# Yeicor/sdf-viewer

Hardware: AMD Instinct MI355X
Metric: Mvoxels/s grid fill + Mrays/s sphere-trace @1080p, demo SDF (higher is better)
Workload: dtype f32

## Files before the change

sdf-viewer_amd/csrc/api_march.hip:

```cpp
#include <cmath>
#include <cstddef>
#include <cstring>

#include "api_internal.h"
#include "march_common.h"
#include "raymarch_kernels.h"

using namespace sdfv;

namespace {

struct BatchStreams {
    static constexpr int kSide = 3;
    hipStream_t side[kSide] = {};
    hipEvent_t fork = nullptr, join[kSide] = {};
    int device = -1;
    void release() {
        for (int i = 0; i < kSide; ++i) {
            if (side[i]) (void)hipStreamDestroy(side[i]);
            if (join[i]) (void)hipEventDestroy(join[i]);
        }
        if (fork) (void)hipEventDestroy(fork);
        *this = BatchStreams{};
    }
    hipError_t ensure(int device_now) {
        if (device == device_now && fork) return hipSuccess;
        release();
        hipError_t e = hipEventCreateWithFlags(&fork, hipEventDisableTiming);
        for (int i = 0; i < kSide && e == hipSuccess; ++i) {
            e = hipStreamCreateWithFlags(&side[i], hipStreamNonBlocking);
            if (e == hipSuccess) e = hipEventCreateWithFlags(&join[i], hipEventDisableTiming);
        }
        if (e != hipSuccess) release();
        else device = device_now;
        return e;
    }
};
thread_local BatchStreams g_batch_streams;

struct CameraRing {
    static constexpr uint32_t kSlots = 16;
    sdfv_camera* base = nullptr;
    hipEvent_t read[kSlots] = {};
    bool recorded[kSlots] = {};
    uint32_t next = 0;
    int device = -1;
    void release() {
        for (uint32_t i = 0; i < kSlots; ++i)
            if (read[i]) (void)hipEventDestroy(read[i]);
        if (base) (void)hipFree(base);
        *this = CameraRing{};
    }
    hipError_t ensure(int device_now) {
        if (device == device_now && base) return hipSuccess;
        release();
        hipError_t e = hipMalloc(reinterpret_cast<void**>(&base), (size_t)kSlots * sdfv::kMaxCamerasPerLaunch * sizeof(sdfv_camera));
        for (uint32_t i = 0; i < kSlots && e == hipSuccess; ++i) e = hipEventCreateWithFlags(&read[i], hipEventDisableTiming);
        if (e != hipSuccess) {
            (void)hipGetLastError();
            release();
        } else {
            device = device_now;
        }
        return e;
    }
};
thread_local CameraRing g_camera_ring;

}

namespace sdfv {
void release_march_caches() {
    g_batch_streams.release();
    g_camera_ring.release();
}

int check_lights(const sdfv_render_params* rp) {
    if (rp->n_lights > SDFV_MAX_LIGHTS)
        return set_error(SDFV_ERR_INVALID_ARGUMENT, "n_lights %u exceeds SDFV_MAX_LIGHTS", rp->n_lights);
    for (uint32_t i = 0; i < rp->n_lights; ++i) {
        if (rp->lights[i].kind == SDFV_LIGHT_DIRECTIONAL)
            return set_error(SDFV_ERR_INVALID_ARGUMENT,
                        "lights[%u] is directional: three-d 0.18.2 shader source not available (scene/mod.rs:107-112 keeps "
                        "its directional lights commented out; their BRDF is not restated from memory)", i);
        if (rp->lights[i].kind != SDFV_LIGHT_AMBIENT)
            return set_error(SDFV_ERR_INVALID_ARGUMENT, "lights[%u] has unknown kind %u", i, rp->lights[i].kind);
    }
    return SDFV_OK;
}
}

namespace {

void derive_raymarch_args(const sdfv_render_params* rp, sdfv::RaymarchArgs& a) {
    memset(&a, 0, sizeof(a));
    a.rp = *rp;
    const uint32_t off = g_options.raymarch_disable;
    a.pow2_extent = (off & SDFV_RM_NO_POW2_EXTENT) ? 0u : 1u;
    a.fast_index = (off & SDFV_RM_NO_FAST_INDEX) ? 0u : 1u;
    a.pow2_size = 1;
    a.symmetric_box = 1;
    a.fast_normal = 1;
    float radius2 = 0.0f;
    const float h_world = sdfv::march::tap_distance((float)rp->tex_size[0], (float)rp->tex_size[1], (float)rp->tex_size[2],
                                                    rp->lod_dist_between_samples);
    for (int i = 0; i < 3; ++i) {
        a.bsize[i] = rp->bounds_max[i] - rp->bounds_min[i];
        a.inv_bsize[i] = 1.0f / a.bsize[i];
        const float n = (float)rp->tex_size[i];
        if (!(a.bsize[i] > 0.0f) || !(1e-4f * n / a.bsize[i] <= 0.25f)) a.fast_index = 0;
        if (!(a.bsize[i] > 0.0f) || !((1e-4f + h_world) * n / a.bsize[i] <= 0.45f)) a.fast_normal = 0;
        int e = 0;
        if (!(a.bsize[i] > 0.0f) || frexpf(a.bsize[i], &e) != 0.5f || e < -100 || e > 100) a.pow2_extent = 0;
        if (rp->tex_size[i] >= (1u << 24)) a.pow2_size = 0;
        if (rp->bounds_min[i] != -rp->bounds_max[i]) a.symmetric_box = 0;
        a.cull_center[i] = 0.5f * (rp->bounds_min[i] + rp->bounds_max[i]);
        radius2 += 0.25f * a.bsize[i] * a.bsize[i];
    }
    a.cull_radius2 = radius2 * 1.0201f + 1e-12f;
    if (!(a.cull_radius2 > 0.0f) || !std::isfinite(a.cull_radius2)) a.cull_radius2 = INFINITY;
    a.asm_loop = (off & SDFV_RM_NO_ASM_LOOP) ? 0u : 1u;
    a.no_interior_fetch = (off & SDFV_RM_NO_INTERIOR_FETCH) ? 1u : 0u;
    a.cube_box = (a.symmetric_box && rp->bounds_max[0] == rp->bounds_max[1] && rp->bounds_max[1] == rp->bounds_max[2]) ? 1u : 0u;
    if (off & SDFV_RM_NO_SYMMETRIC) a.symmetric_box = 0;
    if (off & SDFV_RM_NO_POW2_SIZE) a.pow2_size = 0;
}

void set_march_frame(sdfv::RaymarchArgs& a, const float* tex0, const float* tex1, uint32_t width, uint32_t height, uint32_t y0, uint32_t y1) {
    a.tex0 = reinterpret_cast<const float4*>(tex0);
    a.tex1 = reinterpret_cast<const float4*>(tex1);
    a.width = width;
    a.height = height;
    a.y0 = y0;
    a.y1 = y1;
}

int raymarch_rows(const sdfv_march_desc& d, uint32_t y0, uint32_t y1, uint32_t band_step, uint32_t band_height, void* stream) {
    const sdfv_render_params* rp = d.rp;
    const uint32_t n_cameras = d.n_cameras, width = d.width, height = d.height;
    const sdfv_camera* cameras = d.cameras;
    if (!rp || !d.tex0 || !d.tex1) return set_error(SDFV_ERR_INVALID_ARGUMENT, "NULL argument");
    if (!d.rgba && !d.rgba8) return set_error(SDFV_ERR_INVALID_ARGUMENT, "no colour output: rgba and rgba8 are both NULL");
    if (int rc = check_lights(rp)) return rc;
    if (int rc = check_texel_alignment(d.tex0, d.tex1, d.rgba)) return rc;
    if (int rc = check_word_aligned("dist, depth, aux and rgba8", d.dist, d.depth, d.aux, d.rgba8)) return rc;
    if (((uintptr_t)d.pairs | (uintptr_t)d.ilv) & 7) return set_error(SDFV_ERR_INVALID_ARGUMENT, "pairs and ilv must be 8-byte aligned");
    if (n_cameras && !cameras) return set_error(SDFV_ERR_INVALID_ARGUMENT, "cameras is NULL");
    if (y0 > y1 || y1 > height) return set_error(SDFV_ERR_INVALID_ARGUMENT, "rows [%u,%u) outside height %u", y0, y1, height);
    if (rp->tex_size[0] == 0 || rp->tex_size[1] == 0 || rp->tex_size[2] == 0)
        return set_error(SDFV_ERR_INVALID_ARGUMENT, "empty texture");
    if (!(rp->lod_dist_between_samples >= 1.0f)) return set_error(SDFV_ERR_INVALID_ARGUMENT, "lod_dist_between_samples < 1");
    const uint32_t lod_filter = g_options.raymarch_lod_filter;
    if (lod_filter == 1 && rp->lod_dist_between_samples != 1.0f) {
        int e = 0;
        const float lod = rp->lod_dist_between_samples;
        if (!(lod >= 2.0f && lod <= 32768.0f) || frexpf(lod, &e) != 0.5f)
            return set_error(SDFV_ERR_INVALID_ARGUMENT,
                             "SDFV_OPT_RAYMARCH_LOD_FILTER 1: lod_dist_between_samples %g is not a power of two in [2, 32768]", (double)lod);
    }
    if ((uint64_t)rp->tex_size[0] * rp->tex_size[1] * rp->tex_size[2] >= (1ull << 32))
        return set_error(SDFV_ERR_INVALID_ARGUMENT, "texture too large for 32-bit texel indexing");
    if (int rc = need_device()) return rc;
    sdfv::RaymarchArgs a;
    derive_raymarch_args(rp, a);
    a.dist = d.dist;
    a.pairs = d.pairs;
    a.ilv = d.ilv;
    set_march_frame(a, d.tex0, d.tex1, width, height, y0, y1);
    a.band_skip = band_height * (band_step - 1u);
    a.band_shift = band_height == 8u ? 3u : 4u;
    a.rows_out = band_step > 1 ? sdfv_band_rows_ex(height, y0 / band_height, band_step, band_height) : y1 - y0;
    a.compute_normal = g_options.raymarch_keep_normal ? 1u : 0u;
    const uint32_t w = g_options.raymarch_waves_per_simd;
    a.waves_per_simd = w;
    a.box_first = g_options.raymarch_box_first;
    const DeviceFacts& dev = device_facts();
    if (!dev.gfx950) a.asm_loop = 0;
    a.wave_slots_per_simd_unit = dev.cus * 4u;
    a.last_level_cache_bytes = dev.last_level_cache_bytes;
    const bool xcd_order_ok = dev.xcds == 8;
    a.group_shift = g_options.raymarch_tile_group == 0 ? (n_cameras == 1 && xcd_order_ok ? sdfv::kGroupAuto : 0u)
                                                       : (g_options.raymarch_tile_group == 1 ? 0u : g_options.raymarch_tile_group - 1u);
    a.rotate_columns = g_options.raymarch_tile_group == 0 && xcd_order_ok ? 1u : 0u;
#ifdef SDFV_TUNING
    a.wave_timing = reinterpret_cast<unsigned long long*>(g_options.wave_timing);
    a.priority_map = reinterpret_cast<const unsigned char*>(g_options.priority_map);
    a.tile_order = n_cameras == 1 ? reinterpret_cast<const uint32_t*>(g_options.tile_order) : nullptr;
#endif
    const uint64_t pixels_per_cam = (uint64_t)a.rows_out * width;
    hipStream_t main = (hipStream_t)stream;
    const sdfv_camera* device_cameras = nullptr;
    bool ring = false;
    hipPointerAttribute_t attr;
    if (hipPointerGetAttributes(&attr, cameras) == hipSuccess && (attr.type == hipMemoryTypeDevice || attr.type == hipMemoryTypeManaged)) {
        device_cameras = cameras;
    } else {
        (void)hipGetLastError();
        if (n_cameras > sdfv::kInlineCameras) {
            hipStreamCaptureStatus capturing = hipStreamCaptureStatusNone;
            if (hipStreamIsCapturing(main, &capturing) != hipSuccess) (void)hipGetLastError();
            ring = capturing == hipStreamCaptureStatusNone && g_options.raymarch_camera_staging &&
                   g_camera_ring.ensure(current_device()) == hipSuccess;
        }
    }
    const uint32_t per_launch = device_cameras || ring ? sdfv::kMaxCamerasPerLaunch : sdfv::kInlineCameras;
    const uint64_t groups_per_launch = (uint64_t)((width + 15) / 16) * ((a.rows_out + 15) / 16) * per_launch;
    const bool overlap = n_cameras > per_launch && groups_per_launch <= 40000 && g_options.raymarch_batch_streams;
    uint32_t used = 0;
    int rc = SDFV_OK;
    auto hip_ok = [&](hipError_t e, const char* what) {
        if (e != hipSuccess && rc == SDFV_OK) rc = hip_fail(e, what);
        return e == hipSuccess;
    };
    if (overlap) hip_ok(g_batch_streams.ensure(current_device()), "batch streams") && hip_ok(hipEventRecord(g_batch_streams.fork, main), "hipEventRecord");
    uint32_t launch = 0;
    for (uint32_t c0 = 0; c0 < n_cameras && rc == SDFV_OK; c0 += per_launch, ++launch) {
        const uint32_t nc = n_cameras - c0 < per_launch ? n_cameras - c0 : per_launch;
        a.n_cameras = nc;
        if (device_cameras) a.camera_list = device_cameras + c0;
        else if (!ring) memcpy(a.cameras, cameras + c0, nc * sizeof(sdfv_camera));
        point_outputs_at(a, pixels_per_cam, c0, d.rgba, d.rgba8, d.aux, d.depth);
        hipStream_t on = main;
        const uint32_t lane = launch % (BatchStreams::kSide + 1);
        if (overlap && lane != 0) {
            on = g_batch_streams.side[lane - 1];
            if (lane > used) {
                if (!hip_ok(hipStreamWaitEvent(on, g_batch_streams.fork, 0), "hipStreamWaitEvent")) break;
                used = lane;
            }
        }
        if (ring) {
            CameraRing& r = g_camera_ring;
            const uint32_t slot = r.next++ % CameraRing::kSlots;
            sdfv_camera* at = r.base + (size_t)slot * sdfv::kMaxCamerasPerLaunch;
            if (r.recorded[slot] && !hip_ok(hipStreamWaitEvent(on, r.read[slot], 0), "hipStreamWaitEvent")) break;
            if (!hip_ok(sdfv::launch_store_cameras(cameras + c0, nc, at, on), "store_cameras")) break;
            a.camera_list = at;
            hip_ok(sdfv::launch_raymarch(a, on, lod_filter), "launch_raymarch") && hip_ok(hipEventRecord(r.read[slot], on), "hipEventRecord");
            r.recorded[slot] = true;
            continue;
        }
        hip_ok(sdfv::launch_raymarch(a, on, lod_filter), "launch_raymarch");
    }
    for (uint32_t i = 0; i < used; ++i)
        hip_ok(hipEventRecord(g_batch_streams.join[i], g_batch_streams.side[i]), "hipEventRecord") &&
            hip_ok(hipStreamWaitEvent(main, g_batch_streams.join[i], 0), "hipStreamWaitEvent");
    return rc;
}

int slab_round_args(const sdfv_render_params* rp, const sdfv_grid* slab, uint32_t ghost_lo, uint32_t ghost_hi,
                           const float* tex0, const float* tex1, const sdfv_camera* camera, uint32_t width, uint32_t height,
                           float* rgba, sdfv_march_aux* aux, sdfv::RaymarchArgs& a, sdfv::SlabMarchArgs& s) {
    if (!rp || !slab || !tex0 || !tex1 || !camera || !rgba) return set_error(SDFV_ERR_INVALID_ARGUMENT, "NULL argument");
    if (int rc = check_grid(slab)) return rc;
    if (int rc = check_lights(rp)) return rc;
    if (int rc = check_texel_alignment(tex0, tex1, rgba)) return rc;
    for (int i = 0; i < 3; ++i)
        if (rp->tex_size[i] != slab->dims[i])
            return set_error(SDFV_ERR_INVALID_ARGUMENT, "render parameters describe a %ux%ux%u grid, the slab a %ux%ux%u one",
                        rp->tex_size[0], rp->tex_size[1], rp->tex_size[2], slab->dims[0], slab->dims[1], slab->dims[2]);
    if (slab->z_begin >= slab->z_end) return set_error(SDFV_ERR_INVALID_ARGUMENT, "empty slab");
    if (ghost_lo > slab->z_begin || slab->z_end + ghost_hi > slab->dims[2])
        return set_error(SDFV_ERR_INVALID_ARGUMENT, "ghost slices reach outside the grid");
    if (ghost_lo > 1 || ghost_hi > 2) return set_error(SDFV_ERR_INVALID_ARGUMENT, "at most 1 lower and 2 upper ghost slices");
    if (slab->z_end < slab->dims[2] && ghost_hi == 0)
        return set_error(SDFV_ERR_INVALID_ARGUMENT, "an interior slab needs its upper ghost slice (run the halo exchange)");
    if (rp->lod_dist_between_samples != 1.0f)
        return set_error(SDFV_ERR_INVALID_ARGUMENT, "the sharded march renders loaded grids only (lod_dist_between_samples == 1)");
    if ((uint64_t)width * height >= (1ull << 32)) return set_error(SDFV_ERR_INVALID_ARGUMENT, "image too large");
    const uint64_t resident = (uint64_t)slab->dims[0] * slab->dims[1] * (ghost_lo + (slab->z_end - slab->z_begin) + ghost_hi);
    if (resident >= (1ull << 32)) return set_error(SDFV_ERR_INVALID_ARGUMENT, "slab too large for 32-bit texel indexing");
    if (int rc = need_device()) return rc;
    derive_raymarch_args(rp, a);
    if (!a.fast_index)
        return set_error(SDFV_ERR_INVALID_ARGUMENT, "box too small for the sharded march: 1e-4 * N / size must be <= 0.25");
    set_march_frame(a, tex0, tex1, width, height, 0, height);
    a.rows_out = height;
    a.band_shift = 4;
    a.n_cameras = 1;
    a.cameras[0] = *camera;
    a.rgba = reinterpret_cast<float4*>(rgba);
    a.aux = aux;
    s = sdfv::SlabMarchArgs{};
    s.z_lo = slab->z_begin - ghost_lo;
    s.z_count = ghost_lo + (slab->z_end - slab->z_begin) + ghost_hi;
    s.own_begin = slab->z_begin;
    s.own_end = slab->z_end;
    return SDFV_OK;
}

}

#pragma GCC visibility push(default)
extern "C" {

void sdfv_render_params_default(sdfv_render_params* rp, const sdfv_grid* grid) {
    if (!rp) return;
    memset(rp, 0, sizeof(*rp));
    for (int i = 0; i < 3; ++i) {
        if (grid) {
            rp->bounds_min[i] = grid->bb_min[i];
            rp->bounds_max[i] = grid->bb_max[i];
            rp->tex_size[i] = grid->dims[i];
        }
        rp->ambient[i] = 1.0f;
    }
    rp->lod_dist_between_samples = 1.0f;
    rp->tint[0] = rp->tint[1] = rp->tint[2] = rp->tint[3] = 1.0f;
    rp->gamma = 0.0f;
    rp->tone_mapping = 2;
    rp->color_mapping = 1;
}

int sdfv_march_volume_advice(const sdfv_grid* grid, uint32_t* kind) {
    if (int rc = check_grid(grid)) return rc;
    if (!kind) return set_error(SDFV_ERR_INVALID_ARGUMENT, "kind is NULL");
    if (int rc = need_device()) return rc;
    sdfv_render_params rp;
    sdfv_render_params_default(&rp, grid);
    sdfv::RaymarchArgs a;
    derive_raymarch_args(&rp, a);
    if (!device_facts().gfx950) a.asm_loop = 0;
    a.last_level_cache_bytes = device_facts().last_level_cache_bytes;
    const int mode = sdfv::march_volume_choice(a, true, true, true);
    *kind = mode == sdfv::kMarchIlv ? SDFV_MARCH_VOLUME_INTERLEAVED : mode == sdfv::kMarchPairs ? SDFV_MARCH_VOLUME_PAIRS : SDFV_MARCH_VOLUME_NONE;
    return SDFV_OK;
}

int sdfv_raymarch_ex(const sdfv_march_desc* desc, void* stream) {
    sdfv_march_desc d;
    if (int rc = read_sized_desc(desc, offsetof(sdfv_march_desc, depth), "sdfv_march_desc", d)) return rc;
    if (d.reserved != 0) return set_error(SDFV_ERR_INVALID_ARGUMENT, "sdfv_march_desc: reserved fields must be 0");
    if (d.band_step == 0 && d.band_height != 0)
        return set_error(SDFV_ERR_INVALID_ARGUMENT, "band_height %u with band_step 0: a band set needs band_step >= 1 (0 = rows [y0, y1))", d.band_height);
    if (d.band_step == 0)
        return raymarch_rows(d, d.y0, d.y1, 1, 16, stream);
    const uint32_t B = d.band_height ? d.band_height : 16u;
    if (B != 8u && B != 16u) return set_error(SDFV_ERR_INVALID_ARGUMENT, "band_height %u: 8 or 16 (0 = 16)", d.band_height);
    if (sdfv_band_rows_ex(d.height, d.band_first, d.band_step, B) == 0) return SDFV_OK;
    return raymarch_rows(d, d.band_first * B, d.height, d.band_step, B, stream);
}

uint32_t sdfv_band_rows_ex(uint32_t height, uint32_t band_first, uint32_t band_step, uint32_t band_height) {
    const uint32_t B = band_height ? band_height : 16u;
    if (B != 8u && B != 16u) return 0;
    const uint32_t bands = (height + B - 1) / B;
    if (band_step == 0 || band_first >= bands) return 0;
    const uint32_t n = (bands - band_first + band_step - 1) / band_step, last = band_first + (n - 1) * band_step;
    return (n - 1) * B + (height - last * B < B ? height - last * B : B);
}
uint32_t sdfv_band_rows(uint32_t height, uint32_t band_first, uint32_t band_step) {
    return sdfv_band_rows_ex(height, band_first, band_step, 16u);
}

int sdfv_raymarch_slab(const sdfv_render_params* rp, const sdfv_grid* slab, uint32_t ghost_lo, uint32_t ghost_hi,
                       const float* tex0, const float* tex1, const sdfv_camera* camera, uint32_t width, uint32_t height,
                       const sdfv_ray_state* in_states, uint32_t n_in, float* rgba, sdfv_march_aux* aux,
                       sdfv_ray_state* out_down, sdfv_ray_state* out_up, uint32_t capacity, uint32_t* counters,
                       void* stream) {
    if (!out_down || !out_up || !counters) return set_error(SDFV_ERR_INVALID_ARGUMENT, "NULL argument");
    if (in_states == nullptr && n_in != 0) return set_error(SDFV_ERR_INVALID_ARGUMENT, "n_in without in_states");
    sdfv::RaymarchArgs a;
    sdfv::SlabMarchArgs s;
    if (int rc = slab_round_args(rp, slab, ghost_lo, ghost_hi, tex0, tex1, camera, width, height, rgba, aux, a, s)) return rc;
    s.in = in_states;
    s.n_in = n_in;
    s.out_down = out_down;
    s.out_up = out_up;
    s.count_down = counters;
    s.count_up = counters + 1;
    s.capacity = capacity;
    if (in_states && n_in == 0) return SDFV_OK;
    SDFV_HIP_RETURN(sdfv::launch_raymarch_slab(a, s, (hipStream_t)stream));
}

size_t sdfv_ray_buffer_bytes(uint32_t capacity) { return SDFV_RAY_BUFFER_HEADER_BYTES + (size_t)capacity * sizeof(sdfv_ray_state); }

int sdfv_raymarch_slab_round(const sdfv_render_params* rp, const sdfv_grid* slab, uint32_t ghost_lo, uint32_t ghost_hi,
                             const float* tex0, const float* tex1, const sdfv_camera* camera, uint32_t width, uint32_t height,
                             const void* in_lo, const void* in_hi, int first_round, float* rgba, sdfv_march_aux* aux,
                             void* out_down, void* out_up, uint32_t capacity, uint32_t* overflow, void* stream) {
    return sdfv_internal_raymarch_slab_round(rp, slab, ghost_lo, ghost_hi, tex0, tex1, camera, width, height, in_lo, in_hi,
                                             first_round, rgba, aux, out_down, out_up, capacity, overflow, nullptr, stream);
}

__attribute__((visibility("hidden"))) int sdfv_internal_raymarch_slab_round(
    const sdfv_render_params* rp, const sdfv_grid* slab, uint32_t ghost_lo, uint32_t ghost_hi, const float* tex0, const float* tex1,
    const sdfv_camera* camera, uint32_t width, uint32_t height, const void* in_lo, const void* in_hi, int first_round, float* rgba,
    sdfv_march_aux* aux, void* out_down, void* out_up, uint32_t capacity, uint32_t* overflow, uint32_t* leftover, void* stream) {
    if (!out_down || !out_up) return set_error(SDFV_ERR_INVALID_ARGUMENT, "NULL ray buffer");
    if (int rc = check_word_aligned("ray buffers", in_lo, in_hi, out_down, out_up, overflow)) return rc;
    if (first_round && (in_lo || in_hi)) return set_error(SDFV_ERR_INVALID_ARGUMENT, "the first round takes no incoming rays");
    sdfv::RaymarchArgs a;
    sdfv::SlabMarchArgs s;
    if (int rc = slab_round_args(rp, slab, ghost_lo, ghost_hi, tex0, tex1, camera, width, height, rgba, aux, a, s)) return rc;
    auto count_of = [](const void* b) { return reinterpret_cast<const uint32_t*>(b); };
    auto rays_of = [](const void* b) {
        return reinterpret_cast<const sdfv_ray_state*>(static_cast<const char*>(b) + SDFV_RAY_BUFFER_HEADER_BYTES);
    };
    SDFV_HIP(hipMemsetAsync(out_down, 0, SDFV_RAY_BUFFER_HEADER_BYTES, (hipStream_t)stream));
    SDFV_HIP(hipMemsetAsync(out_up, 0, SDFV_RAY_BUFFER_HEADER_BYTES, (hipStream_t)stream));
    if (!first_round) {
        if (!in_lo && !in_hi) return SDFV_OK;
        s.in_count[0] = in_lo ? count_of(in_lo) : nullptr;
        s.in_rays[0] = in_lo ? rays_of(in_lo) : nullptr;
        s.in_count[1] = in_hi ? count_of(in_hi) : nullptr;
        s.in_rays[1] = in_hi ? rays_of(in_hi) : nullptr;
        const uint64_t most = (uint64_t)capacity * ((in_lo ? 1u : 0u) + (in_hi ? 1u : 0u));
        const uint64_t pixels = (uint64_t)width * height;
        s.max_in = (uint32_t)(most < pixels ? most : pixels);
        if (s.max_in == 0) return SDFV_OK;
    }
    s.out_down = const_cast<sdfv_ray_state*>(rays_of(out_down));
    s.out_up = const_cast<sdfv_ray_state*>(rays_of(out_up));
    s.count_down = reinterpret_cast<uint32_t*>(out_down);
    s.count_up = reinterpret_cast<uint32_t*>(out_up);
    s.overflow = overflow;
    s.leftover = leftover;
    s.capacity = capacity;
    SDFV_HIP_RETURN(sdfv::launch_raymarch_slab(a, s, (hipStream_t)stream));
}

}
#pragma GCC visibility pop
```

sdf-viewer_amd/csrc/raymarch_kernels.h:

```cpp
#pragma once

#include <hip/hip_runtime.h>
#include <stdint.h>

#include "../../include/sdfgrid.h"

namespace sdfv {

struct RaymarchArgs {
    sdfv_render_params rp;
    float bsize[3];
    float inv_bsize[3];
    uint32_t pow2_extent;
    uint32_t fast_index;
    const float* dist;
    const float* pairs;
    const float* ilv;
    uint32_t pow2_size;
    uint32_t symmetric_box;
    uint32_t fast_normal;
    float cull_center[3];
    float cull_radius2;
    const float4* tex0;
    const float4* tex1;
    uint32_t n_cameras;
    uint32_t width, height;
    uint32_t y0, y1;
    uint32_t compute_normal;
    uint32_t asm_loop;
    uint32_t group_shift;
    uint32_t tiles_x, tiles_y, groups_x;
    uint32_t box_first;
    uint32_t first_gx0, first_gy0, first_w, first_h, m_groups_x, m_first_w, m_rest_w;
    uint32_t no_interior_fetch;
    uint32_t rotate_columns;
    uint32_t lds_cap_bytes;
    uint32_t waves_per_simd;
    uint32_t wave_slots_per_simd_unit;
    uint64_t last_level_cache_bytes;
    uint32_t cube_box;
    uint32_t rows_out;
    uint32_t band_skip;
    uint32_t band_shift;
    float4* rgba;
    uint32_t* rgba8;
    sdfv_march_aux* aux;
    float* depth;
#ifdef SDFV_TUNING
    const uint32_t* tile_order;
    const unsigned char* priority_map;
    unsigned long long* wave_timing;
#endif
    const sdfv_camera* camera_list;
    sdfv_camera cameras[16];
};

constexpr int kMarchGeneral = 0, kMarchTex0 = 1, kMarchDist = 2, kMarchPairs = 3, kMarchIlv = 4, kMarchLattice = 5;

constexpr uint32_t kInlineCameras = 16;
constexpr uint32_t kMaxCamerasPerLaunch = 64;
constexpr uint32_t kGroupAuto = 255;

struct SlabMarchArgs {
    uint32_t z_lo, z_count;
    uint32_t own_begin, own_end;
    const sdfv_ray_state* in;
    uint32_t n_in;
    const uint32_t* in_count[2];
    const sdfv_ray_state* in_rays[2];
    uint32_t max_in;
    sdfv_ray_state* out_down;
    sdfv_ray_state* out_up;
    uint32_t* count_down;
    uint32_t* count_up;
    uint32_t* overflow;
    uint32_t* leftover;
    uint32_t capacity;
};
hipError_t launch_raymarch_slab(const RaymarchArgs& a, const SlabMarchArgs& s, hipStream_t stream);

hipError_t launch_raymarch(const RaymarchArgs& a, hipStream_t stream, uint32_t lod_filter);
bool march_volume_applicable(const RaymarchArgs& a, int kind);
int march_volume_choice(const RaymarchArgs& a, bool have_dist, bool have_pairs, bool have_ilv);
hipError_t launch_store_cameras(const sdfv_camera* host, uint32_t n, sdfv_camera* device, hipStream_t stream);

}
```

sdf-viewer_amd/csrc/raymarch_kernels.hip:

```cpp
#include "raymarch_kernels.h"

#include <hip/hip_runtime.h>
#include <string.h>

#include "march_common.h"

namespace sdfv {
namespace {

using namespace march;

__device__ __forceinline__ uint32_t mirror_index(int i, int n) {
    if (i >= 0 && i < n) return (uint32_t)i;
    int period = 2 * n;
    int m = i % period;
    if (m < 0) m += period;
    return (uint32_t)(m < n ? m : period - 1 - m);
}

struct Tex {
    const float4* data;
    int w, h, d;
    int z_lo;
};

struct Footprint {
    uint32_t o000, o100, o010, o110, o001, o101, o011, o111;
    float ax, ay, az;
};

constexpr int kMirror = 0, kClamp = 1, kClampSlab = 2;

template <int POLICY>
__device__ __forceinline__ Footprint footprint(const Tex& t, V3 p01, int& k0c) {
    float u = p01.x * (float)t.w - 0.5f, v = p01.y * (float)t.h - 0.5f, w = p01.z * (float)t.d - 0.5f;
    float fu = floorf(u), fv = floorf(v), fw = floorf(w);
    Footprint f;
    f.ax = u - fu; f.ay = v - fv; f.az = w - fw;
    int i0 = (int)fu, j0 = (int)fv, k0 = (int)fw;
    uint32_t i0m, i1m, j0m, j1m, k0m, k1m;
    const uint32_t sy = (uint32_t)t.w, sz = (uint32_t)t.w * (uint32_t)t.h;
    k0c = 0;
    if (POLICY == kMirror) {
        i0m = mirror_index(i0, t.w); i1m = mirror_index(i0 + 1, t.w);
        j0m = mirror_index(j0, t.h) * sy; j1m = mirror_index(j0 + 1, t.h) * sy;
        k0m = mirror_index(k0, t.d) * sz; k1m = mirror_index(k0 + 1, t.d) * sz;
    } else {
        const int z0 = POLICY == kClampSlab ? t.z_lo : 0;
        i0m = (uint32_t)max(i0, 0); i1m = (uint32_t)min(i0 + 1, t.w - 1);
        j0m = (uint32_t)max(j0, 0) * sy; j1m = (uint32_t)min(j0 + 1, t.h - 1) * sy;
        k0c = min(max(k0, 0), t.d - 1);
        k0m = (uint32_t)(max(k0, 0) - z0) * sz; k1m = (uint32_t)(min(k0 + 1, t.d - 1) - z0) * sz;
    }
    f.o000 = k0m + j0m + i0m; f.o100 = k0m + j0m + i1m;
    f.o010 = k0m + j1m + i0m; f.o110 = k0m + j1m + i1m;
    f.o001 = k1m + j0m + i0m; f.o101 = k1m + j0m + i1m;
    f.o011 = k1m + j1m + i0m; f.o111 = k1m + j1m + i1m;
    return f;
}

__device__ __forceinline__ float trilerp(float t000, float t100, float t010, float t110, float t001, float t101,
                                         float t011, float t111, float ax, float ay, float az) {
    float c00 = mixf(t000, t100, ax), c10 = mixf(t010, t110, ax);
    float c01 = mixf(t001, t101, ax), c11 = mixf(t011, t111, ax);
    return mixf(mixf(c00, c10, ay), mixf(c01, c11, ay), az);
}

template <int POLICY>
__device__ __forceinline__ Footprint footprint(const Tex& t, V3 p01) {
    int k0c;
    return footprint<POLICY>(t, p01, k0c);
}

__device__ __forceinline__ float gather_r(const float* base, uint32_t stride, const Footprint& f) {
    const float t000 = base[(uint64_t)f.o000 * stride], t100 = base[(uint64_t)f.o100 * stride];
    const float t010 = base[(uint64_t)f.o010 * stride], t110 = base[(uint64_t)f.o110 * stride];
    const float t001 = base[(uint64_t)f.o001 * stride], t101 = base[(uint64_t)f.o101 * stride];
    const float t011 = base[(uint64_t)f.o011 * stride], t111 = base[(uint64_t)f.o111 * stride];
    return trilerp(t000, t100, t010, t110, t001, t101, t011, t111, f.ax, f.ay, f.az);
}

__device__ __forceinline__ float4 gather_rgba(const float4* data, const Footprint& f) {
    const float4 t000 = data[f.o000], t100 = data[f.o100], t010 = data[f.o010], t110 = data[f.o110];
    const float4 t001 = data[f.o001], t101 = data[f.o101], t011 = data[f.o011], t111 = data[f.o111];
    float4 r;
    r.x = trilerp(t000.x, t100.x, t010.x, t110.x, t001.x, t101.x, t011.x, t111.x, f.ax, f.ay, f.az);
    r.y = trilerp(t000.y, t100.y, t010.y, t110.y, t001.y, t101.y, t011.y, t111.y, f.ax, f.ay, f.az);
    r.z = trilerp(t000.z, t100.z, t010.z, t110.z, t001.z, t101.z, t011.z, t111.z, f.ax, f.ay, f.az);
    r.w = trilerp(t000.w, t100.w, t010.w, t110.w, t001.w, t101.w, t011.w, t111.w, f.ax, f.ay, f.az);
    return r;
}

template <int XF>
__device__ __forceinline__ V3 to_p01(const RaymarchArgs& a, V3 p) {
    if (XF >= 1)
        return mk((p.x - a.rp.bounds_min[0]) * a.inv_bsize[0], (p.y - a.rp.bounds_min[1]) * a.inv_bsize[1],
                  (p.z - a.rp.bounds_min[2]) * a.inv_bsize[2]);
    return mk((p.x - a.rp.bounds_min[0]) / a.bsize[0], (p.y - a.rp.bounds_min[1]) / a.bsize[1],
              (p.z - a.rp.bounds_min[2]) / a.bsize[2]);
}

__device__ __forceinline__ uint32_t nearest_offset(const RaymarchArgs& a, const Tex& t, V3 p01) {
    float rx = (float)t.w / a.rp.lod_dist_between_samples;
    float ry = (float)t.h / a.rp.lod_dist_between_samples;
    float rz = (float)t.d / a.rp.lod_dist_between_samples;
    float qx = roundf(p01.x * rx) / rx, qy = roundf(p01.y * ry) / ry, qz = roundf(p01.z * rz) / rz;
    int i = (int)floorf(qx * (float)t.w), j = (int)floorf(qy * (float)t.h), k = (int)floorf(qz * (float)t.d);
    return (mirror_index(k, t.d) * (uint32_t)t.h + mirror_index(j, t.h)) * (uint32_t)t.w + mirror_index(i, t.w);
}

template <bool LINEAR, int XF, int POLICY>
__device__ __forceinline__ float sample_r(const RaymarchArgs& a, const float* __restrict__ base, uint32_t stride, const Tex& t, V3 p) {
    V3 q = to_p01<XF>(a, p);
    if (LINEAR) return gather_r(base, stride, footprint<POLICY>(t, q));
    return base[(uint64_t)nearest_offset(a, t, q) * stride];
}

template <bool LINEAR, int XF, int POLICY>
__device__ __forceinline__ float4 sample_rgba(const RaymarchArgs& a, const Tex& t, V3 p) {
    V3 q = to_p01<XF>(a, p);
    if (LINEAR) return gather_rgba(t.data, footprint<POLICY>(t, q));
    return t.data[nearest_offset(a, t, q)];
}

template <bool SYMM>
__device__ __forceinline__ float oob_dist(const RaymarchArgs& a, V3 p) {
    if (SYMM) {
        return fmaxf(fabsf(p.x) - a.rp.bounds_max[0],
                     fmaxf(fabsf(p.y) - a.rp.bounds_max[1], fabsf(p.z) - a.rp.bounds_max[2]));
    }
    return march::oob_dist(a.rp, p);
}

template <int MODE>
__device__ __forceinline__ const float* march_volume(const RaymarchArgs& a) {
    return MODE == kMarchTex0 ? reinterpret_cast<const float*>(a.tex0) : MODE == kMarchDist ? a.dist : MODE == kMarchPairs ? a.pairs : a.ilv;
}

template <int MODE, int XF, bool SYMM, bool T>
__device__ __forceinline__ void march_fast(const RaymarchArgs& a, const Tex& t, V3 ray_dir, bool covered, V3& ray_pos,
                                           float& dist_from_origin, int& status, int& steps, int& iterations) {
    static_assert(MODE == kMarchTex0 || MODE == kMarchDist, "the pair and interleaved volumes are read by the hand-written loop only");
    constexpr int STRIDE = MODE == kMarchTex0 ? 4 : 1;
    const float* __restrict__ vol = march_volume<MODE>(a);
    const float fw_ = (float)t.w, fh_ = (float)t.h, fd_ = (float)t.d;
    const float kx = a.inv_bsize[0] * fw_, ky = a.inv_bsize[1] * fh_, kz = a.inv_bsize[2] * fd_;
    const int wm1 = t.w - 1, hm1 = t.h - 1, dm1 = t.d - 1;
    const uint32_t sy = (uint32_t)t.w, sz = (uint32_t)t.w * (uint32_t)t.h;
    bool marching = covered;
    int last_i = -1;
    float cfu = -4.0f, cfv = -4.0f, cfw = -4.0f;
    float t000 = 0.0f, t100 = 0.0f, t010 = 0.0f, t110 = 0.0f, t001 = 0.0f, t101 = 0.0f, t011 = 0.0f, t111 = 0.0f;
    for (int i = 0; i < 255; ++i) {
        marching = marching && !(oob_dist<SYMM>(a, ray_pos) > 1e-4f);
        if (__ballot(marching) == 0ull) break;
        ++iterations;
        last_i = marching ? i : last_i;
        float u, v, w;
        if (XF == 2) {
            u = (ray_pos.x - a.rp.bounds_min[0]) * kx - 0.5f;
            v = (ray_pos.y - a.rp.bounds_min[1]) * ky - 0.5f;
            w = (ray_pos.z - a.rp.bounds_min[2]) * kz - 0.5f;
        } else {
            const V3 q = to_p01<XF>(a, ray_pos);
            u = q.x * fw_ - 0.5f; v = q.y * fh_ - 0.5f; w = q.z * fd_ - 0.5f;
        }
        const float fu = floorf(u), fv = floorf(v), fw = floorf(w);
        const float ax = u - fu, ay = v - fv, az = w - fw;
        if (marching && (fu != cfu || fv != cfv || fw != cfw)) {
            cfu = fu; cfv = fv; cfw = fw;
            const int i0 = (int)fu, j0 = (int)fv, k0 = (int)fw;
            const uint32_t i0c = (uint32_t)max(i0, 0), i1c = (uint32_t)min(i0 + 1, wm1);
            const uint32_t j0c = (uint32_t)max(j0, 0) * sy, j1c = (uint32_t)min(j0 + 1, hm1) * sy;
            const uint32_t k0c = (uint32_t)max(k0, 0) * sz, k1c = (uint32_t)min(k0 + 1, dm1) * sz;
            const uint32_t r00 = k0c + j0c, r10 = k0c + j1c, r01 = k1c + j0c, r11 = k1c + j1c;
            if (STRIDE == 1 && wm1 >= 1) {
                const uint32_t b = (uint32_t)min(max(i0, 0), wm1 - 1);
                const bool lo_is_x = i0c == b, hi_is_y = i1c == b + 1;
                typedef float f2 __attribute__((ext_vector_type(2), aligned(4)));
                const f2 q00 = *reinterpret_cast<const f2*>(vol + (uint64_t)(r00 + b));
                const f2 q10 = *reinterpret_cast<const f2*>(vol + (uint64_t)(r10 + b));
                const f2 q01 = *reinterpret_cast<const f2*>(vol + (uint64_t)(r01 + b));
                const f2 q11 = *reinterpret_cast<const f2*>(vol + (uint64_t)(r11 + b));
                t000 = lo_is_x ? q00.x : q00.y; t100 = hi_is_y ? q00.y : q00.x;
                t010 = lo_is_x ? q10.x : q10.y; t110 = hi_is_y ? q10.y : q10.x;
                t001 = lo_is_x ? q01.x : q01.y; t101 = hi_is_y ? q01.y : q01.x;
                t011 = lo_is_x ? q11.x : q11.y; t111 = hi_is_y ? q11.y : q11.x;
            } else {
                t000 = vol[(uint64_t)(r00 + i0c) * STRIDE]; t100 = vol[(uint64_t)(r00 + i1c) * STRIDE];
                t010 = vol[(uint64_t)(r10 + i0c) * STRIDE]; t110 = vol[(uint64_t)(r10 + i1c) * STRIDE];
                t001 = vol[(uint64_t)(r01 + i0c) * STRIDE]; t101 = vol[(uint64_t)(r01 + i1c) * STRIDE];
                t011 = vol[(uint64_t)(r11 + i0c) * STRIDE]; t111 = vol[(uint64_t)(r11 + i1c) * STRIDE];
            }
        }
        const float sample_dist = trilerp(t000, t100, t010, t110, t001, t101, t011, t111, ax, ay, az) - 1e-1f;
        marching = marching && !(sample_dist < 1e-5f);
        const V3 np = madd(ray_pos, ray_dir, sample_dist);
        ray_pos.x = marching ? np.x : ray_pos.x;
        ray_pos.y = marching ? np.y : ray_pos.y;
        ray_pos.z = marching ? np.z : ray_pos.z;
        if (T) {
            const float nt = dist_from_origin + sample_dist;
            dist_from_origin = marching ? nt : dist_from_origin;
        }
    }
    steps = last_i + 1;
    if (covered) status = marching ? -1 : (oob_dist<SYMM>(a, ray_pos) > 1e-4f ? -2 : 1);
}

struct Lattice {
    uint32_t shift;
    float inv_l;
    int mx1, my1, mz1;
};
__device__ __forceinline__ Lattice lattice_of(const RaymarchArgs& a, const Tex& t) {
    const uint32_t l = (uint32_t)a.rp.lod_dist_between_samples;
    Lattice g;
    g.shift = 31u - (uint32_t)__builtin_clz(l);
    g.inv_l = 1.0f / a.rp.lod_dist_between_samples;
    g.mx1 = (int)(((uint32_t)t.w + l - 1u) >> g.shift) - 1;
    g.my1 = (int)(((uint32_t)t.h + l - 1u) >> g.shift) - 1;
    g.mz1 = (int)(((uint32_t)t.d + l - 1u) >> g.shift) - 1;
    return g;
}
__device__ __forceinline__ void lattice_cell(const Tex& t, const Lattice& g, float fu, float fv, float fw, Footprint& f) {
    const int i0 = (int)fu, j0 = (int)fv, k0 = (int)fw;
    const uint32_t sy = (uint32_t)t.w, sz = (uint32_t)t.w * (uint32_t)t.h;
    const uint32_t i0m = (uint32_t)min(max(i0, 0), g.mx1) << g.shift, i1m = (uint32_t)min(max(i0 + 1, 0), g.mx1) << g.shift;
    const uint32_t j0m = ((uint32_t)min(max(j0, 0), g.my1) << g.shift) * sy, j1m = ((uint32_t)min(max(j0 + 1, 0), g.my1) << g.shift) * sy;
    const uint32_t k0m = ((uint32_t)min(max(k0, 0), g.mz1) << g.shift) * sz, k1m = ((uint32_t)min(max(k0 + 1, 0), g.mz1) << g.shift) * sz;
    f.o000 = k0m + j0m + i0m; f.o100 = k0m + j0m + i1m;
    f.o010 = k0m + j1m + i0m; f.o110 = k0m + j1m + i1m;
    f.o001 = k1m + j0m + i0m; f.o101 = k1m + j0m + i1m;
    f.o011 = k1m + j1m + i0m; f.o111 = k1m + j1m + i1m;
}
__device__ __forceinline__ Footprint lattice_footprint(const Tex& t, const Lattice& g, V3 p01) {
    const float u = p01.x * (float)t.w - 0.5f, v = p01.y * (float)t.h - 0.5f, w = p01.z * (float)t.d - 0.5f;
    const float su = u * g.inv_l, sv = v * g.inv_l, sw = w * g.inv_l;
    const float fu = floorf(su), fv = floorf(sv), fw = floorf(sw);
    Footprint f;
    f.ax = su - fu; f.ay = sv - fv; f.az = sw - fw;
    lattice_cell(t, g, fu, fv, fw, f);
    return f;
}

template <int XF, bool SYMM, bool T>
__device__ __forceinline__ void march_lattice(const RaymarchArgs& a, const Tex& t, const Lattice& g, V3 ray_dir, bool covered, V3& ray_pos,
                                              float& dist_from_origin, int& status, int& steps, int& iterations) {
    static_assert(XF == 0 || XF == 1, "no fused scale: s = (q * N - 0.5) / L keeps the LINEAR footprint's u");
    const float* __restrict__ vol = reinterpret_cast<const float*>(a.tex0);
    const float fw_ = (float)t.w, fh_ = (float)t.h, fd_ = (float)t.d;
    bool marching = covered;
    int last_i = -1;
    float cfu = __int_as_float(0x7fc00000), cfv = cfu, cfw = cfu;
    float t000 = 0.0f, t100 = 0.0f, t010 = 0.0f, t110 = 0.0f, t001 = 0.0f, t101 = 0.0f, t011 = 0.0f, t111 = 0.0f;
    for (int i = 0; i < 255; ++i) {
        marching = marching && !(oob_dist<SYMM>(a, ray_pos) > 1e-4f);
        if (__ballot(marching) == 0ull) break;
        ++iterations;
        last_i = marching ? i : last_i;
        const V3 q = to_p01<XF>(a, ray_pos);
        const float su = (q.x * fw_ - 0.5f) * g.inv_l, sv = (q.y * fh_ - 0.5f) * g.inv_l, sw = (q.z * fd_ - 0.5f) * g.inv_l;
        const float fu = floorf(su), fv = floorf(sv), fw = floorf(sw);
        const float ax = su - fu, ay = sv - fv, az = sw - fw;
        if (marching && (fu != cfu || fv != cfv || fw != cfw)) {
            cfu = fu; cfv = fv; cfw = fw;
            Footprint c;
            lattice_cell(t, g, fu, fv, fw, c);
            t000 = vol[(uint64_t)c.o000 * 4]; t100 = vol[(uint64_t)c.o100 * 4];
            t010 = vol[(uint64_t)c.o010 * 4]; t110 = vol[(uint64_t)c.o110 * 4];
            t001 = vol[(uint64_t)c.o001 * 4]; t101 = vol[(uint64_t)c.o101 * 4];
            t011 = vol[(uint64_t)c.o011 * 4]; t111 = vol[(uint64_t)c.o111 * 4];
        }
        const float sample_dist = trilerp(t000, t100, t010, t110, t001, t101, t011, t111, ax, ay, az) - 1e-1f;
        marching = marching && !(sample_dist < 1e-5f);
        const V3 np = madd(ray_pos, ray_dir, sample_dist);
        ray_pos.x = marching ? np.x : ray_pos.x;
        ray_pos.y = marching ? np.y : ray_pos.y;
        ray_pos.z = marching ? np.z : ray_pos.z;
        if (T) {
            const float nt = dist_from_origin + sample_dist;
            dist_from_origin = marching ? nt : dist_from_origin;
        }
    }
    steps = last_i + 1;
    if (covered) status = marching ? -1 : (oob_dist<SYMM>(a, ray_pos) > 1e-4f ? -2 : 1);
}

#ifdef SDFV_TUNING
#define SDFV_MARCH_ASM_TUNE(x) x
#else
#define SDFV_MARCH_ASM_TUNE(x) ""
#endif
#define SDFV_MARCH_ASM_HEAD(ROW_BYTES)                                                                                         \
    "s_mov_b64 s[76:77], exec\n"                                                                                    \
    "s_and_b64 exec, exec, %[cov]\n"                                                                                \
    "s_cbranch_execz .Ldone_%=\n"                                                                                   \
          \
    "s_mov_b32 s66, %[miny]\n s_mov_b32 s67, %[minz]\n"                                            \
    "s_mov_b32 s70, %[ky]\n s_mov_b32 s71, %[kz]\n"                                                    \
    "s_mov_b32 s72, 0xbf000000\n s_mov_b32 s73, 0xbf000000\n"                                      \
    "s_add_i32 s75, %[wm1], -1\n"                                                                         \
    "s_lshl_b32 s82, %[w], 2\n s_lshl_b32 s83, %[w], 4\n"         \
    "s_lshl_b32 s85, %[w], 3\n"                                      \
    "s_movk_i32 s74, 254\n"                                                                      \
     \
    "s_mov_b32 s64, " ROW_BYTES "\n"                                                                                 \
    "s_mul_i32 s86, %[h], " ROW_BYTES "\n"                                                                           \
    "s_add_u32 s68, %[base_lo], s86\n s_addc_u32 s69, %[base_hi], 0\n"                                      \
    "s_add_u32 s64, %[base_lo], s64\n s_addc_u32 s65, %[base_hi], 0\n"                                      \
    "s_add_u32 s86, s64, s86\n s_addc_u32 s87, s65, 0\n"                                                    \
    SDFV_MARCH_ASM_TUNE("s_mov_b32 s84, 0\n")                  \
    "v_mov_b32 v68, 0x7f800000\n v_mov_b32 v70, 0x7f800000\n v_mov_b32 v71, 0x7f800000\n"     \
    ".Lloop_%=:\n"
#define SDFV_MARCH_ASM_OOB4_A "v_sub_f32_e64 v32, |v40|, %[mx]\n"
#define SDFV_MARCH_ASM_OOB4_B "v_sub_f32_e64 v33, |v42|, %[my]\n"
#define SDFV_MARCH_ASM_OOB4_C "v_sub_f32_e64 v34, |v43|, %[mz]\n"
#define SDFV_MARCH_ASM_OOB4_D "v_max3_f32 v32, v32, v33, v34\n"
#define SDFV_MARCH_ASM_OOB2_A "v_max3_f32 v32, |v40|, |v42|, |v43|\n"
#define SDFV_MARCH_ASM_OOB2_D "v_subrev_f32_e32 v32, %[mx], v32\n"
#define SDFV_MARCH_ASM_TOP(T_STEP, OOB_A, OOB_B, OOB_C, OOB_D)                                                      \
    OOB_A                                                                                                           \
    "v_subrev_f32_e32 v48, %[minx], v40\n"                                                                          \
    OOB_B                                                                                                           \
    "v_pk_add_f32 v[50:51], v[42:43], s[66:67] neg_lo:[0,1] neg_hi:[0,1]\n"                                         \
    OOB_C                                                                                                           \
    "v_mul_f32_e32 v48, %[kx], v48\n"                                                                               \
    "v_pk_mul_f32 v[50:51], v[50:51], s[70:71]\n"                                                                   \
    OOB_D                                                                                                           \
    "v_add_f32_e32 v48, -0.5, v48\n"                                                                                \
    "v_pk_add_f32 v[50:51], v[50:51], s[72:73]\n"                                                                   \
    "v_cmpx_nlt_f32_e32 vcc, 0x38d1b717, v32\n"                                           \
    "s_cbranch_execz .Ldone_%=\n"                                                                                   \
    "v_sub_f32_e32 v52, v48, v68\n"                                                                              \
    "v_sub_f32_e32 v54, v50, v70\n"                                                                              \
    "v_sub_f32_e32 v56, v51, v71\n" T_STEP                                                                       \
    "v_max3_u32 v32, v52, v54, v56\n"                                                                            \
    "v_cmp_gt_u32_e32 vcc, 0x3f800000, v32\n"                                                                       \
    "s_andn1_saveexec_b64 s[78:79], vcc\n"                                      \
    "s_cbranch_execnz .Lfetch_%=\n"                                  \
    ".Lcached_%=:\n"
#define SDFV_MARCH_ASM_FETCH_PREP(INTERIOR)                                                                         \
    ".Lfetch_%=:\n"                                                                                                 \
    SDFV_MARCH_ASM_TUNE("s_add_u32 s84, s84, 1\n")                                                                  \
        \
    "v_floor_f32_e32 v68, v48\n v_floor_f32_e32 v70, v50\n v_floor_f32_e32 v71, v51\n"                         \
    "v_cvt_i32_f32_e32 v32, v68\n v_cvt_i32_f32_e32 v33, v70\n v_cvt_i32_f32_e32 v34, v71\n"                      \
    "v_sub_f32_e32 v52, v48, v68\n v_sub_f32_e32 v54, v50, v70\n v_sub_f32_e32 v56, v51, v71\n"             \
     \
    "v_max3_u32 v35, v32, v33, v34\n"                                                                               \
    "v_cmp_gt_u32_e32 vcc, %[thresh], v35\n"                                                                        \
    "s_xor_b64 vcc, vcc, exec\n"                                                                                    \
    "s_cbranch_scc1 .Lborder_%=\n"                                                                                  \
    "v_mad_u32_u24 v39, v34, %[h], v33\n"                     \
    "v_mad_u32_u24 v39, v39, %[w], v32\n" INTERIOR                                                               \
    "s_branch .Lcached_%=\n"                                                                                        \
    ".Lborder_%=:\n"                                                                                                \
    "v_max_i32_e32 v35, 0, v32\n v_max_i32_e32 v37, 0, v33\n v_max_i32_e32 v38, 0, v34\n"         \
    "v_add_u32_e32 v32, 1, v32\n v_add_u32_e32 v33, 1, v33\n v_add_u32_e32 v34, 1, v34\n"                            \
    "v_min_i32_e32 v32, %[wm1], v32\n v_min_i32_e32 v33, %[hm1], v33\n v_min_i32_e32 v34, %[dm1], v34\n"   \
    "v_mad_u32_u24 v28, v38, %[h], v37\n"                                                      \
    "v_mad_u32_u24 v29, v38, %[h], v33\n"                                                      \
    "v_mad_u32_u24 v30, v34, %[h], v37\n"                                                      \
    "v_mad_u32_u24 v31, v34, %[h], v33\n"
#define SDFV_MARCH_ASM_INTERIOR_DIST                                                                                \
    "v_lshlrev_b32_e32 v39, 2, v39\n"                                                                               \
    "global_load_dwordx2 v[24:25], v39, %[base]\n"                                        \
    "global_load_dwordx2 v[26:27], v39, s[64:65]\n"                                       \
    "global_load_dwordx2 v[28:29], v39, s[68:69]\n"                                       \
    "global_load_dwordx2 v[30:31], v39, s[86:87]\n"                                       \
    "s_waitcnt vmcnt(1)\n"                                                                                          \
    "v_pk_mov_b32 v[60:61], v[24:25], v[28:29] op_sel:[0,0]\n"                                    \
    "v_pk_mov_b32 v[62:63], v[24:25], v[28:29] op_sel:[1,1]\n"                                    \
    "s_waitcnt vmcnt(0)\n"                                                                                          \
    "v_pk_mov_b32 v[64:65], v[26:27], v[30:31] op_sel:[0,0]\n"                                    \
    "v_pk_mov_b32 v[66:67], v[26:27], v[30:31] op_sel:[1,1]\n"
#define SDFV_MARCH_ASM_INTERIOR_TEX0                                                                                \
    "v_lshlrev_b32_e32 v39, 4, v39\n"                                                                               \
    "global_load_dword v60, v39, %[base]\n global_load_dword v62, v39, %[base] offset:16\n"                       \
    "global_load_dword v64, v39, s[64:65]\n global_load_dword v66, v39, s[64:65] offset:16\n"                     \
    "global_load_dword v61, v39, s[68:69]\n global_load_dword v63, v39, s[68:69] offset:16\n"                     \
    "global_load_dword v65, v39, s[86:87]\n global_load_dword v67, v39, s[86:87] offset:16\n"                     \
    "s_waitcnt vmcnt(0)\n"
#define SDFV_MARCH_ASM_INTERIOR_PAIRS                                                                               \
    "v_lshlrev_b32_e32 v39, 3, v39\n"                                                                               \
    "global_load_dwordx4 v[24:27], v39, %[base]\n"                                  \
    "global_load_dwordx4 v[28:31], v39, s[68:69]\n"                                 \
    "s_waitcnt vmcnt(0)\n"                                                                                          \
    "v_pk_mov_b32 v[60:61], v[24:25], v[28:29] op_sel:[0,0]\n"                                    \
    "v_pk_mov_b32 v[64:65], v[24:25], v[28:29] op_sel:[1,1]\n"                                    \
    "v_pk_mov_b32 v[62:63], v[26:27], v[30:31] op_sel:[0,0]\n"                                    \
    "v_pk_mov_b32 v[66:67], v[26:27], v[30:31] op_sel:[1,1]\n"
#define SDFV_MARCH_ASM_FETCH_PAIRS                                                                                  \
    "v_lshlrev_b32_e32 v35, 3, v35\n v_lshlrev_b32_e32 v32, 3, v32\n"                  \
    "v_mad_u32_u24 v24, v28, s85, v35\n v_mad_u32_u24 v25, v28, s85, v32\n"                                          \
    "global_load_dword v60, v24, %[base]\n global_load_dword v62, v25, %[base]\n"                                  \
    "v_mad_u32_u24 v26, v29, s85, v35\n v_mad_u32_u24 v27, v29, s85, v32\n"                                          \
    "global_load_dword v64, v26, %[base]\n global_load_dword v66, v27, %[base]\n"                                  \
    "v_mad_u32_u24 v24, v30, s85, v35\n v_mad_u32_u24 v25, v30, s85, v32\n"                                          \
    "global_load_dword v61, v24, %[base]\n global_load_dword v63, v25, %[base]\n"                                  \
    "v_mad_u32_u24 v26, v31, s85, v35\n v_mad_u32_u24 v27, v31, s85, v32\n"                                          \
    "global_load_dword v65, v26, %[base]\n global_load_dword v67, v27, %[base]\n"                                  \
    "s_waitcnt vmcnt(0)\n"                                                                                          \
    "s_branch .Lcached_%=\n"
#define SDFV_MARCH_ASM_INTERIOR_ILV                                                                                 \
    "s_lshr_b32 s80, %[h], 1\n"                                                                                     \
    "v_and_b32_e32 v48, 1, v33\n"                                                                  \
    "v_lshrrev_b32_e32 v35, 1, v33\n"                                                              \
    "v_add_u32_e32 v36, 1, v33\n"                                                                                   \
    "v_lshrrev_b32_e32 v36, 1, v36\n"                                                        \
    "v_mad_u32_u24 v35, v34, s80, v35\n v_mad_u32_u24 v36, v34, s80, v36\n"              \
    "v_mad_u32_u24 v35, v35, %[w], v32\n v_mad_u32_u24 v37, v36, %[w], v32\n"                                        \
    "v_lshlrev_b32_e32 v36, 3, v35\n v_lshlrev_b32_e32 v37, 3, v37\n"                                               \
    "v_cmp_eq_u32_e32 vcc, 1, v48\n"                                                                                \
    "global_load_dwordx4 v[24:27], v36, %[base]\n"                      \
    "global_load_dwordx4 v[32:35], v36, s[68:69]\n"                                                      \
    "s_and_saveexec_b64 s[80:81], vcc\n"                      \
    "global_load_dwordx3 v[28:30], v37, %[base]\n"                                   \
    "global_load_dwordx3 v[36:38], v37, s[68:69]\n"                                                      \
    "s_mov_b64 exec, s[80:81]\n"                                                                                    \
    "s_waitcnt vmcnt(2)\n"                                                                                          \
    "v_cndmask_b32_e32 v60, v24, v25, vcc\n v_cndmask_b32_e32 v62, v26, v27, vcc\n"          \
    "v_cndmask_b32_e32 v61, v32, v33, vcc\n v_cndmask_b32_e32 v63, v34, v35, vcc\n"                  \
    "s_waitcnt vmcnt(0)\n"                                                                                          \
    "v_cndmask_b32_e32 v64, v25, v28, vcc\n v_cndmask_b32_e32 v66, v27, v30, vcc\n"      \
    "v_cndmask_b32_e32 v65, v33, v36, vcc\n v_cndmask_b32_e32 v67, v35, v38, vcc\n"
#define SDFV_MARCH_ASM_ILV_ROW(R)                             \
    "v_and_b32_e32 v36, 1, v" #R "\n"                                                                     \
    "v_lshrrev_b32_e32 v" #R ", 1, v" #R "\n"                                     \
    "v_mul_u32_u24_e32 v" #R ", s85, v" #R "\n"                                                         \
    "v_lshl_add_u32 v" #R ", v36, 2, v" #R "\n"
#define SDFV_MARCH_ASM_FETCH_ILV                                                                                    \
    "v_lshlrev_b32_e32 v35, 3, v35\n v_lshlrev_b32_e32 v32, 3, v32\n"         \
    SDFV_MARCH_ASM_ILV_ROW(28) SDFV_MARCH_ASM_ILV_ROW(29) SDFV_MARCH_ASM_ILV_ROW(30) SDFV_MARCH_ASM_ILV_ROW(31)       \
    "v_add_u32_e32 v24, v28, v35\n v_add_u32_e32 v25, v28, v32\n"                                                    \
    "global_load_dword v60, v24, %[base]\n global_load_dword v62, v25, %[base]\n"                                  \
    "v_add_u32_e32 v26, v29, v35\n v_add_u32_e32 v27, v29, v32\n"                                                    \
    "global_load_dword v64, v26, %[base]\n global_load_dword v66, v27, %[base]\n"                                  \
    "v_add_u32_e32 v24, v30, v35\n v_add_u32_e32 v25, v30, v32\n"                                                    \
    "global_load_dword v61, v24, %[base]\n global_load_dword v63, v25, %[base]\n"                                  \
    "v_add_u32_e32 v26, v31, v35\n v_add_u32_e32 v27, v31, v32\n"                                                    \
    "global_load_dword v65, v26, %[base]\n global_load_dword v67, v27, %[base]\n"                                  \
    "s_waitcnt vmcnt(0)\n"                                                                                          \
    "s_branch .Lcached_%=\n"
#define SDFV_MARCH_ASM_FETCH_DIST                                                                                   \
    "v_min_i32_e32 v36, s75, v35\n"                                                         \
    "v_lshlrev_b32_e32 v39, 2, v36\n"                                                                               \
    "v_mad_u32_u24 v28, v28, s82, v39\n v_mad_u32_u24 v29, v29, s82, v39\n"                                          \
    "v_mad_u32_u24 v30, v30, s82, v39\n v_mad_u32_u24 v31, v31, s82, v39\n"                                          \
    "global_load_dwordx2 v[24:25], v28, %[base]\n"                                                     \
    "global_load_dwordx2 v[26:27], v29, %[base]\n"                                                     \
    "global_load_dwordx2 v[28:29], v30, %[base]\n"                                                     \
    "global_load_dwordx2 v[30:31], v31, %[base]\n"                                                     \
    "v_cmp_eq_u32_e64 s[80:81], v35, v36\n"                                                             \
    "v_add_u32_e32 v36, 1, v36\n"                                                                                   \
    "v_cmp_eq_u32_e32 vcc, v32, v36\n"                                                                  \
    "s_waitcnt vmcnt(3)\n"                                                                                          \
    "v_cndmask_b32_e64 v60, v25, v24, s[80:81]\n v_cndmask_b32_e32 v62, v24, v25, vcc\n"           \
    "s_waitcnt vmcnt(2)\n"                                                                                          \
    "v_cndmask_b32_e64 v64, v27, v26, s[80:81]\n v_cndmask_b32_e32 v66, v26, v27, vcc\n"           \
    "s_waitcnt vmcnt(1)\n"                                                                                          \
    "v_cndmask_b32_e64 v61, v29, v28, s[80:81]\n v_cndmask_b32_e32 v63, v28, v29, vcc\n"           \
    "s_waitcnt vmcnt(0)\n"                                                                                          \
    "v_cndmask_b32_e64 v65, v31, v30, s[80:81]\n v_cndmask_b32_e32 v67, v30, v31, vcc\n"           \
    "s_branch .Lcached_%=\n"
#define SDFV_MARCH_ASM_FETCH_TEX0                                                                                   \
    "v_lshlrev_b32_e32 v35, 4, v35\n v_lshlrev_b32_e32 v32, 4, v32\n"                  \
    "v_mad_u32_u24 v24, v28, s83, v35\n v_mad_u32_u24 v25, v28, s83, v32\n"                                          \
    "global_load_dword v60, v24, %[base]\n global_load_dword v62, v25, %[base]\n"                                  \
    "v_mad_u32_u24 v26, v29, s83, v35\n v_mad_u32_u24 v27, v29, s83, v32\n"                                          \
    "global_load_dword v64, v26, %[base]\n global_load_dword v66, v27, %[base]\n"                                  \
    "v_mad_u32_u24 v24, v30, s83, v35\n v_mad_u32_u24 v25, v30, s83, v32\n"                                          \
    "global_load_dword v61, v24, %[base]\n global_load_dword v63, v25, %[base]\n"                                  \
    "v_mad_u32_u24 v26, v31, s83, v35\n v_mad_u32_u24 v27, v31, s83, v32\n"                                          \
    "global_load_dword v65, v26, %[base]\n global_load_dword v67, v27, %[base]\n"                                  \
    "s_waitcnt vmcnt(0)\n"                                                                                          \
    "s_branch .Lcached_%=\n"
#define SDFV_MARCH_ASM_FILTER                                                                                       \
    "s_mov_b64 exec, s[78:79]\n"                                                                                    \
    "v_sub_f32_e32 v53, 1.0, v52\n v_sub_f32_e32 v55, 1.0, v54\n v_sub_f32_e32 v57, 1.0, v56\n"                \
                                                                \
    "v_pk_mul_f32 v[34:35], v[62:63], v[52:53] op_sel_hi:[1,0]\n"                                                \
    "v_pk_mul_f32 v[38:39], v[66:67], v[52:53] op_sel_hi:[1,0]\n"                                                \
    "v_pk_mul_f32 v[32:33], v[60:61], v[52:53] op_sel:[0,1] op_sel_hi:[1,1]\n"                                   \
    "v_pk_mul_f32 v[36:37], v[64:65], v[52:53] op_sel:[0,1] op_sel_hi:[1,1]\n"                                   \
    "v_pk_add_f32 v[32:33], v[32:33], v[34:35]\n"                                                    \
    "v_pk_add_f32 v[36:37], v[36:37], v[38:39]\n"                                                    \
                                                                                                   \
    "v_pk_mul_f32 v[32:33], v[32:33], v[54:55] op_sel:[0,1] op_sel_hi:[1,1]\n"                                     \
    "v_pk_mul_f32 v[36:37], v[36:37], v[54:55] op_sel_hi:[1,0]\n"                                                  \
    "v_pk_add_f32 v[32:33], v[32:33], v[36:37]\n"                                                      \
                                                                       \
    "v_pk_mul_f32 v[32:33], v[32:33], v[56:57] op_sel:[0,1] op_sel_hi:[1,0]\n"       \
    "v_add_f32_e32 v36, v32, v33\n"                                                                                 \
    "v_add_f32_e32 v36, 0xbdcccccd, v36\n"                                                                          \
                                                                                 \
    "v_cmpx_ngt_f32_e32 vcc, 0x3727c5ac, v36\n"
#define SDFV_MARCH_ASM_ADVANCE                                                                                      \
                                                           \
    "v_mul_f32_e32 v32, v44, v36\n"                                                                                \
    "v_pk_mul_f32 v[34:35], v[46:47], v[36:37] op_sel_hi:[1,0]\n"                                                  \
    "v_add_f32_e32 v40, v40, v32\n"                                                                                 \
    "v_pk_add_f32 v[42:43], v[42:43], v[34:35]\n"                                                                   \
    "s_add_u32 s74, s74, -1\n"                                                    \
    "s_cbranch_scc1 .Lloop_%=\n"                                                                                    \
    "s_branch .Ldone_%=\n"
#define SDFV_MARCH_ASM_EPILOGUE                                                                                     \
    ".Ldone_%=:\n"                                                                                                  \
    "s_mov_b64 %[ran], exec\n"                                        \
    "s_mov_b32 %[left], s74\n"                                                                                      \
    SDFV_MARCH_ASM_TUNE("s_lshl_b32 s84, s84, 16\n s_and_b32 %[left], %[left], 0xffff\n s_or_b32 %[left], %[left], s84\n") \
    "s_and_b64 exec, s[76:77], %[cov]\n"                                                                            \
    "s_nop 0\n"
#define SDFV_MARCH_ASM_END "s_mov_b64 exec, s[76:77]\n"
#define SDFV_MARCH_ASM_OPERANDS                                                                                     \
    [dx] "v"(dirx), [dy] "v"(diry), [dz] "v"(dirz), [cov] "s"(cov), [mx] "s"(a.rp.bounds_max[0]),    \
        [my] "s"(a.rp.bounds_max[1]), [mz] "s"(a.rp.bounds_max[2]), [minx] "s"(a.rp.bounds_min[0]),                 \
        [miny] "s"(a.rp.bounds_min[1]), [minz] "s"(a.rp.bounds_min[2]), [kx] "s"(kx), [ky] "s"(ky), [kz] "s"(kz),   \
        [wm1] "s"(wm1), [hm1] "s"(hm1), [dm1] "s"(dm1), [w] "s"(t.w), [h] "s"(t.h), [base] "s"(vol), [base_lo] "s"(base_lo), [base_hi] "s"(base_hi), [thresh] "s"(thresh)
#define SDFV_MARCH_ASM_CLOBBERS                                                                                     \
    "vcc", "scc", "memory", "s64", "s65", "s66", "s67", "s68", "s69", "s70", "s71", "s72", "s73", "s74", "s75",    \
        "s76", "s77", "s78", "s79", "s80", "s81", "s82", "s83", "s84", "s85", "s86", "s87", "v24", "v25", "v26", "v27", "v28",  \
        "v29", "v30", "v31", "v32", "v33", "v34", "v35", "v36", "v37", "v38", "v39", "v48", "v50", "v51", "v52",    \
        "v53", "v54", "v55", "v56", "v57", "v58", "v59", "v60", "v61", "v62", "v63", "v64", "v65", "v66", "v67", "v68",   \
        "v70", "v71"

template <int MODE, bool T>
__device__ __forceinline__ void march_asm(const RaymarchArgs& a, const Tex& t, V3 ray_dir, bool covered, V3& ray_pos,
                                          float& dist_from_origin, int& status, int& steps, int& iterations) {
    const float* __restrict__ vol = march_volume<MODE>(a);
    auto uniform = [](float f) { return __int_as_float(__builtin_amdgcn_readfirstlane(__float_as_int(f))); };
    const float kx = uniform(a.inv_bsize[0] * (float)t.w), ky = uniform(a.inv_bsize[1] * (float)t.h),
                kz = uniform(a.inv_bsize[2] * (float)t.d);
    const int wm1 = t.w - 1, hm1 = t.h - 1, dm1 = t.d - 1;
    const unsigned long long cov = __ballot(covered);
    const uint32_t base_lo = (uint32_t)(uintptr_t)vol, base_hi = (uint32_t)((uintptr_t)vol >> 32);
    const uint32_t thresh = (t.w == t.h && t.h == t.d && !a.no_interior_fetch) ? (uint32_t)t.w - 1u : 0u;
    unsigned long long ran_out;
    int left = 254;
    register float px asm("v40") = ray_pos.x;
    register float py asm("v42") = ray_pos.y;
    register float pz asm("v43") = ray_pos.z;
    register float dirx asm("v44") = ray_dir.x;
    register float diry asm("v46") = ray_dir.y;
    register float dirz asm("v47") = ray_dir.z;
#define SDFV_MARCH_ASM_OOB_BOX SDFV_MARCH_ASM_OOB4_A, SDFV_MARCH_ASM_OOB4_B, SDFV_MARCH_ASM_OOB4_C, SDFV_MARCH_ASM_OOB4_D
#define SDFV_MARCH_ASM_OOB_CUBE SDFV_MARCH_ASM_OOB2_A, "", "", SDFV_MARCH_ASM_OOB2_D
#define SDFV_MARCH_ASM_TOP_(T_STEP, ...) SDFV_MARCH_ASM_TOP(T_STEP, __VA_ARGS__)
#define SDFV_MARCH_ASM_RUN_AUX(SHIFT, INTERIOR, FETCH, OOB)                                                         \
    asm volatile("v_mov_b32 v58, %[tt]\n v_mov_b32 v59, 0\n" SDFV_MARCH_ASM_HEAD(SHIFT)                             \
                 SDFV_MARCH_ASM_TOP_("v_add_u32_e32 v59, 1, v59\n", OOB) SDFV_MARCH_ASM_FILTER                       \
                 "v_add_f32_e32 v58, v58, v36\n" SDFV_MARCH_ASM_ADVANCE SDFV_MARCH_ASM_FETCH_PREP(INTERIOR) FETCH    \
                 SDFV_MARCH_ASM_EPILOGUE "v_mov_b32 %[tt], v58\n v_mov_b32 %[n], v59\n" SDFV_MARCH_ASM_END           \
                 : [px] "+v"(px), [py] "+v"(py), [pz] "+v"(pz), [tt] "+v"(tt), [n] "+v"(n), [ran] "=&s"(ran_out),   \
                   [left] "=&s"(left)                                                                               \
                 : SDFV_MARCH_ASM_OPERANDS                                                                          \
                 : SDFV_MARCH_ASM_CLOBBERS)
#define SDFV_MARCH_ASM_RUN(SHIFT, INTERIOR, FETCH, OOB)                                                             \
    asm volatile(SDFV_MARCH_ASM_HEAD(SHIFT) SDFV_MARCH_ASM_TOP_("", OOB) SDFV_MARCH_ASM_FILTER SDFV_MARCH_ASM_ADVANCE \
                     SDFV_MARCH_ASM_FETCH_PREP(INTERIOR) FETCH SDFV_MARCH_ASM_EPILOGUE SDFV_MARCH_ASM_END            \
                 : [px] "+v"(px), [py] "+v"(py), [pz] "+v"(pz), [ran] "=&s"(ran_out), [left] "=&s"(left)            \
                 : SDFV_MARCH_ASM_OPERANDS                                                                          \
                 : SDFV_MARCH_ASM_CLOBBERS)
#define SDFV_MARCH_ASM_VOL_TEX0 "s83", SDFV_MARCH_ASM_INTERIOR_TEX0, SDFV_MARCH_ASM_FETCH_TEX0
#define SDFV_MARCH_ASM_VOL_DIST "s82", SDFV_MARCH_ASM_INTERIOR_DIST, SDFV_MARCH_ASM_FETCH_DIST
#define SDFV_MARCH_ASM_VOL_PAIRS "s85", SDFV_MARCH_ASM_INTERIOR_PAIRS, SDFV_MARCH_ASM_FETCH_PAIRS
#define SDFV_MARCH_ASM_VOL_ILV "s82", SDFV_MARCH_ASM_INTERIOR_ILV, SDFV_MARCH_ASM_FETCH_ILV
#define SDFV_MARCH_ASM_PER_BOX(RUN, ...)                                                                            \
    if (cube) RUN(__VA_ARGS__, SDFV_MARCH_ASM_OOB_CUBE);                                                            \
    else RUN(__VA_ARGS__, SDFV_MARCH_ASM_OOB_BOX)
#define SDFV_MARCH_ASM_PER_VOLUME(RUN)                                                                              \
    if (MODE == kMarchIlv) { SDFV_MARCH_ASM_PER_BOX(RUN, SDFV_MARCH_ASM_VOL_ILV); }                                 \
    else if (MODE == kMarchPairs) { SDFV_MARCH_ASM_PER_BOX(RUN, SDFV_MARCH_ASM_VOL_PAIRS); }                        \
    else if (MODE == kMarchDist) { SDFV_MARCH_ASM_PER_BOX(RUN, SDFV_MARCH_ASM_VOL_DIST); }                          \
    else { SDFV_MARCH_ASM_PER_BOX(RUN, SDFV_MARCH_ASM_VOL_TEX0); }
    const bool cube = a.cube_box != 0;
    if (T) {
        float tt = dist_from_origin;
        int n = 0;
        SDFV_MARCH_ASM_PER_VOLUME(SDFV_MARCH_ASM_RUN_AUX)
        dist_from_origin = tt;
        steps = n;
    } else {
        SDFV_MARCH_ASM_PER_VOLUME(SDFV_MARCH_ASM_RUN)
    }
#ifdef SDFV_TUNING
    iterations = cov ? (min(255, 255 - (int)(short)(left & 0xffff)) | (left & 0xffff0000)) : 0;
#else
    (void)iterations;
    (void)left;
#endif
    if (covered) {
        ray_pos = mk(px, py, pz);
        const bool ran = ((ran_out >> (threadIdx.x & 63)) & 1ull) != 0;
        status = ran ? -1 : (oob_dist<true>(a, ray_pos) > 1e-4f ? -2 : 1);
    }
}

#ifdef SDFV_TUNING
__device__ __forceinline__ void stamp_wave(const RaymarchArgs& a, uint32_t bx, uint32_t by, uint32_t wave,
                                           unsigned long long t_start, unsigned long long t_start_rt, int iterations,
                                           unsigned long long covered_mask) {
    const uint32_t tiles_x = (a.width + 15) / 16, tiles_y = (a.rows_out + 15) / 16;
    const uint64_t wave_id = ((uint64_t)(blockIdx.z * tiles_y + by) * tiles_x + bx) * 4 + wave;
    a.wave_timing[wave_id * 4 + 0] = t_start;
    a.wave_timing[wave_id * 4 + 1] = __builtin_readcyclecounter();
    a.wave_timing[wave_id * 4 + 2] = (unsigned long long)(uint32_t)iterations | ((t_start_rt & 0xffffull) << 32) |
                                     ((__builtin_amdgcn_s_memrealtime() & 0xffffull) << 48);
    a.wave_timing[wave_id * 4 + 3] = covered_mask;
}
#endif

__device__ __forceinline__ bool box_fragment_ray(const RaymarchArgs& a, V3 eye, V3 d_raw, bool in_image,
                                                 V3& ray_origin, V3& ray_dir) {
    const V3 d0 = normalize(d_raw);
    float tfrag;
    const bool covered = box_slab_test(a.rp, eye, d0, in_image, tfrag);
    fragment_ray(a.rp, eye, d0, tfrag, ray_origin, ray_dir);
    return covered;
}

#ifndef SDFV_RM_MIN_WAVES
#define SDFV_RM_MIN_WAVES 1
#endif
template <int MODE, bool LINEAR, int XF, bool SYMM, bool AUX, bool ASM = false, bool NORMAL = AUX>
__global__ __launch_bounds__(256, SDFV_RM_MIN_WAVES) void raymarch_kernel(RaymarchArgs a) {
    constexpr bool FAST = MODE != 0;
    static_assert(NORMAL || !AUX, "the aux record carries the normal");
#ifdef SDFV_TUNING
    const uint32_t lane = threadIdx.x & 63, wave = threadIdx.x >> 6;
#endif
    uint32_t bx = blockIdx.x, by = blockIdx.y;
#ifdef SDFV_TUNING
    if (a.tile_order) {
        const uint32_t tiles_x = (a.width + 15) / 16, t = a.tile_order[blockIdx.x];
        bx = t % tiles_x;
        by = t / tiles_x;
    } else
#endif
    if (a.group_shift == 0 && a.rotate_columns) {
        const uint32_t tiles_x = gridDim.x;
        const uint32_t r = (blockIdx.y + blockIdx.z) % tiles_x;
        bx = blockIdx.x + r;
        if (bx >= tiles_x) bx -= tiles_x;
    } else if (a.group_shift) {
        const uint32_t g = a.group_shift, per = 1u << (2 * g);
        const uint32_t L = blockIdx.x, xcd = L & 7u, k = L >> 3;
        const uint32_t G = (k >> (2 * g)) * 8u + xcd, t = k & (per - 1u);
        uint32_t gx, gy;
        if (a.first_w == 0) {
            gx = G % a.groups_x;
            gy = G / a.groups_x;
        } else {
            auto div = [](uint32_t n, uint32_t d, uint32_t m) { return d == 1 ? n : __umulhi(n, m); };
            const uint32_t n_in = a.first_w * a.first_h, top = a.first_gy0 * a.groups_x, rest_w = a.groups_x - a.first_w;
            uint32_t j = G - n_in;
            if (G < n_in) {
                const uint32_t r = div(G, a.first_w, a.m_first_w);
                gx = a.first_gx0 + (G - r * a.first_w);
                gy = a.first_gy0 + r;
            } else if (j < top) {
                gy = div(j, a.groups_x, a.m_groups_x);
                gx = j - gy * a.groups_x;
            } else if ((j -= top) < a.first_h * rest_w) {
                const uint32_t r = div(j, rest_w, a.m_rest_w), c = j - r * rest_w;
                gy = a.first_gy0 + r;
                gx = c < a.first_gx0 ? c : c + a.first_w;
            } else {
                j -= a.first_h * rest_w;
                const uint32_t r = div(j, a.groups_x, a.m_groups_x);
                gy = a.first_gy0 + a.first_h + r;
                gx = j - r * a.groups_x;
            }
        }
        bx = (gx << g) + (t & ((1u << g) - 1u));
        by = (gy << g) + (t >> g);
        if (bx >= a.tiles_x || by >= a.tiles_y) return;
    }
    uint32_t px, row;
    tile_pixel(bx, by, px, row);
    const uint32_t py = a.y0 + row + (row >> a.band_shift) * a.band_skip;
    const uint32_t cam_idx = blockIdx.z;
    const bool in_image = px < a.width && py < a.y1;
    sdfv_camera cam;
    if (a.camera_list) cam = a.camera_list[cam_idx];
    else cam = a.cameras[cam_idx];
    const uint64_t out_index = ((uint64_t)cam_idx * a.rows_out + row) * a.width + px;
#ifdef SDFV_TUNING
    if (a.priority_map && a.priority_map[by * ((a.width + 15) / 16) + bx]) __builtin_amdgcn_s_setprio(3);
    const unsigned long long t_start = a.wave_timing ? __builtin_readcyclecounter() : 0ull;
    const unsigned long long t_start_rt = a.wave_timing ? __builtin_amdgcn_s_memrealtime() : 0ull;
#endif

    const V3 eye = mk(cam.eye[0], cam.eye[1], cam.eye[2]);
    const V3 d_raw = pixel_ray_raw(a.width, a.height, cam, px, py);

    {
        const V3 m = sub(eye, mk(a.cull_center[0], a.cull_center[1], a.cull_center[2]));
        const float dd = d_raw.x * d_raw.x + d_raw.y * d_raw.y + d_raw.z * d_raw.z;
        const float mm = m.x * m.x + m.y * m.y + m.z * m.z;
        const float md = m.x * d_raw.x + m.y * d_raw.y + m.z * d_raw.z;
        const float r2 = a.cull_radius2;
        const bool miss = mm > r2 && (md >= 0.0f || mm * dd - md * md > r2 * dd);
        if (__ballot(in_image && !miss) == 0ull) {
            if (in_image) {
                store_color(a, out_index, make_float4(0.0f, 0.0f, 0.0f, 0.0f));
                if (AUX) {
                    sdfv_march_aux aux;
                    aux_clear(aux);
                    a.aux[out_index] = aux;
                }
            }
            if (in_image && a.depth) a.depth[out_index] = 1.0f;
#ifdef SDFV_TUNING
            if (a.wave_timing && lane == 0) stamp_wave(a, bx, by, wave, t_start, t_start_rt, 0, 0ull);
#endif
            return;
        }
    }

    const Tex tex0{a.tex0, (int)a.rp.tex_size[0], (int)a.rp.tex_size[1], (int)a.rp.tex_size[2], 0};
    const Tex tex1{a.tex1, tex0.w, tex0.h, tex0.d, 0};
    const float* tex0_r = reinterpret_cast<const float*>(a.tex0);
    V3 ray_origin, ray_dir;
    const bool covered = box_fragment_ray(a, eye, d_raw, in_image, ray_origin, ray_dir);

    V3 ray_pos = ray_origin;
    float dist_from_origin = 0.0f;
    int status = covered ? -1 : 0;
    int steps = 0;
    int iterations = 0;
#ifdef SDFV_TUNING
    const unsigned long long t_loop0 = a.wave_timing ? __builtin_readcyclecounter() : 0ull;
#endif
    if constexpr (MODE == kMarchLattice) {
        march_lattice<XF, SYMM, AUX>(a, tex0, lattice_of(a, tex0), ray_dir, covered, ray_pos, dist_from_origin, status, steps, iterations);
    } else if constexpr (FAST && ASM) {
        march_asm<MODE, AUX>(a, tex0, ray_dir, covered, ray_pos, dist_from_origin, status, steps, iterations);
    } else if constexpr (FAST) {
        march_fast<MODE, XF, SYMM, AUX>(a, tex0, ray_dir, covered, ray_pos, dist_from_origin, status, steps, iterations);
    } else {
        bool marching = covered;
        for (int i = 0; i < 255; ++i) {
            if (__ballot(marching) == 0ull) break;
            ++iterations;
            if (marching) {
                if (oob_dist<false>(a, ray_pos) > 1e-4f) {
                    status = -2;
                    marching = false;
                } else {
                    float sample_dist = sample_r<LINEAR, XF, kMirror>(a, tex0_r, 4, tex0, ray_pos) - 1e-1f;
                    ++steps;
                    if (sample_dist < 1e-5f) {
                        status = 1;
                        marching = false;
                    } else {
                        dist_from_origin += sample_dist;
                        ray_pos = madd(ray_pos, ray_dir, sample_dist);
                    }
                }
            }
        }
    }

#ifdef SDFV_TUNING
    const unsigned long long t_loop1 = a.wave_timing ? __builtin_readcyclecounter() : 0ull;
#endif
    float4 rgba = make_float4(0.0f, 0.0f, 0.0f, 0.0f);
    float frag_depth = 1.0f;
    sdfv_march_aux aux;
    if (AUX) {
        aux_clear(aux);
        if (covered) aux_set_march(aux, status, steps, ray_pos, dist_from_origin);
    }
    if (status == 1) {
        float4 raw0;
        if constexpr (MODE == kMarchLattice) raw0 = gather_rgba(tex0.data, lattice_footprint(tex0, lattice_of(a, tex0), to_p01<XF>(a, ray_pos)));
        else raw0 = sample_rgba<LINEAR, XF, FAST ? kClamp : kMirror>(a, tex0, ray_pos);
        V3 pos1 = ray_pos;
        asm volatile("" : "+v"(pos1.x) : "v"(raw0.x), "v"(raw0.y), "v"(raw0.z), "v"(raw0.w));
        float4 raw1;
        if constexpr (MODE == kMarchLattice) raw1 = gather_rgba(tex1.data, lattice_footprint(tex1, lattice_of(a, tex1), to_p01<XF>(a, pos1)));
        else raw1 = sample_rgba<LINEAR, XF, FAST ? kClamp : kMirror>(a, tex1, pos1);
        rgba = shade(a.rp, raw0, raw1);
        if (a.depth) {
            frag_depth = frag_depth_of(cam.bvp, ray_pos.x, ray_pos.y, ray_pos.z);
        }
        if (NORMAL) {
            const float h = tap_distance((float)tex0.w, (float)tex0.h, (float)tex0.d, a.rp.lod_dist_between_samples);
            const V3 p1 = normal_tap(ray_pos, h, 0), p2 = normal_tap(ray_pos, h, 1), p3 = normal_tap(ray_pos, h, 2), p4 = normal_tap(ray_pos, h, 3);
            float d1, d2, d3, d4;
            if constexpr (MODE == kMarchLattice) {
                const Lattice g = lattice_of(a, tex0);
                d1 = gather_r(tex0_r, 4, lattice_footprint(tex0, g, to_p01<XF>(a, p1))) - 1e-1f;
                d2 = gather_r(tex0_r, 4, lattice_footprint(tex0, g, to_p01<XF>(a, p2))) - 1e-1f;
                d3 = gather_r(tex0_r, 4, lattice_footprint(tex0, g, to_p01<XF>(a, p3))) - 1e-1f;
                d4 = gather_r(tex0_r, 4, lattice_footprint(tex0, g, to_p01<XF>(a, p4))) - 1e-1f;
            } else if (MODE >= kMarchDist && a.dist && a.fast_normal) {
                d1 = sample_r<true, XF, kClamp>(a, a.dist, 1, tex0, p1) - 1e-1f;
                d2 = sample_r<true, XF, kClamp>(a, a.dist, 1, tex0, p2) - 1e-1f;
                d3 = sample_r<true, XF, kClamp>(a, a.dist, 1, tex0, p3) - 1e-1f;
                d4 = sample_r<true, XF, kClamp>(a, a.dist, 1, tex0, p4) - 1e-1f;
            } else if (FAST && a.fast_normal) {
                d1 = sample_r<LINEAR, XF, kClamp>(a, tex0_r, 4, tex0, p1) - 1e-1f;
                d2 = sample_r<LINEAR, XF, kClamp>(a, tex0_r, 4, tex0, p2) - 1e-1f;
                d3 = sample_r<LINEAR, XF, kClamp>(a, tex0_r, 4, tex0, p3) - 1e-1f;
                d4 = sample_r<LINEAR, XF, kClamp>(a, tex0_r, 4, tex0, p4) - 1e-1f;
            } else {
                d1 = sample_r<LINEAR, XF, kMirror>(a, tex0_r, 4, tex0, p1) - 1e-1f;
                d2 = sample_r<LINEAR, XF, kMirror>(a, tex0_r, 4, tex0, p2) - 1e-1f;
                d3 = sample_r<LINEAR, XF, kMirror>(a, tex0_r, 4, tex0, p3) - 1e-1f;
                d4 = sample_r<LINEAR, XF, kMirror>(a, tex0_r, 4, tex0, p4) - 1e-1f;
            }
            const V3 n = normal_of_taps(d1, d2, d3, d4);
            if (AUX) {
                aux_set_hit(aux, raw0, raw1, n, frag_depth_of(cam.bvp, ray_pos.x, ray_pos.y, ray_pos.z));
            } else {
                asm volatile("" ::"v"(n.x), "v"(n.y), "v"(n.z));
            }
        }
    }

#ifdef SDFV_TUNING
    if (a.wave_timing && lane == 0)
        stamp_wave(a, bx, by, wave, t_start, t_start_rt, iterations, ((t_loop0 - t_start) & 0xffffffffull) | ((t_loop1 - t_loop0) << 32));
#endif
    if (in_image) {
        store_color(a, out_index, rgba);
        if (a.depth) a.depth[out_index] = frag_depth;
        if (AUX) a.aux[out_index] = aux;
    }
}

template <int XF, bool AUX>
__global__ __launch_bounds__(256) void raymarch_slab_kernel(RaymarchArgs a, SlabMarchArgs s) {
    const bool device_counts = s.in_count[0] != nullptr || s.in_count[1] != nullptr;
    const bool first_round = s.in == nullptr && !device_counts;
    const uint32_t gid = blockIdx.x * 256 + threadIdx.x;
    const sdfv_camera& cam = a.cameras[0];
    uint32_t px, py;
    bool live;
    int i = 0;
    V3 ray_pos = mk(0.0f, 0.0f, 0.0f);
    float dist_from_origin = 0.0f;
    if (first_round) {
        const uint32_t tiles_x = (a.width + 7) / 8, tile = gid >> 6, lane = gid & 63;
        px = (tile % tiles_x) * 8 + (lane & 7);
        py = (tile / tiles_x) * 8 + (lane >> 3);
        live = px < a.width && py < a.height;
    } else {
        sdfv_ray_state st{};
        if (device_counts) {
            const uint32_t n0 = s.in_count[0] ? min(*s.in_count[0], s.capacity) : 0u;
            const uint32_t n1 = s.in_count[1] ? min(*s.in_count[1], s.capacity) : 0u;
            live = gid < n0 + n1;
            if (live) st = gid < n0 ? s.in_rays[0][gid] : s.in_rays[1][gid - n0];
        } else {
            live = gid < s.n_in;
            st = s.in[live ? gid : 0];
        }
        if (__ballot(live) == 0ull) return;
        px = st.pixel % a.width;
        py = st.pixel / a.width;
        i = (int)st.iteration;
        ray_pos = mk(st.pos[0], st.pos[1], st.pos[2]);
        dist_from_origin = st.t;
    }
    const uint32_t pixel = py * a.width + px;
    const V3 eye = mk(cam.eye[0], cam.eye[1], cam.eye[2]);
    V3 ray_origin, ray_dir;
    const bool covered = box_fragment_ray(a, eye, pixel_ray_raw(a.width, a.height, cam, px, py), live, ray_origin, ray_dir);
    const Tex tex{a.tex0, (int)a.rp.tex_size[0], (int)a.rp.tex_size[1], (int)a.rp.tex_size[2], (int)s.z_lo};
    const float* dist_r = reinterpret_cast<const float*>(a.tex0);

    bool marching = live && covered;
    if (first_round) {
        ray_pos = ray_origin;
        if (live) {
            a.rgba[pixel] = make_float4(0.0f, 0.0f, 0.0f, 0.0f);
            if (AUX) {
                sdfv_march_aux z;
                aux_clear(z);
                z.depth = 0.0f;
                a.aux[pixel] = z;
            }
        }
        int k0c;
        (void)footprint<kClampSlab>(tex, to_p01<XF>(a, ray_pos), k0c);
        marching = marching && k0c >= (int)s.own_begin && k0c < (int)s.own_end;
    }
    const bool mine = marching;
    int status = 0, steps = 0;
    bool exported = false;
    int export_dir = 0;
    Footprint hit_fp{};
    uint32_t cell0 = 0xffffffffu, cell7 = 0xffffffffu;
    float c000 = 0.0f, c100 = 0.0f, c010 = 0.0f, c110 = 0.0f, c001 = 0.0f, c101 = 0.0f, c011 = 0.0f, c111 = 0.0f;
    for (;;) {
        marching = marching && i < 255;
        if (__ballot(marching) == 0ull) break;
        if (!marching) continue;
        if (oob_dist<false>(a, ray_pos) > 1e-4f) {
            status = -2;
            steps = i;
            marching = false;
            continue;
        }
        int k0c;
        const Footprint f = footprint<kClampSlab>(tex, to_p01<XF>(a, ray_pos), k0c);
        if (k0c < (int)s.own_begin || k0c >= (int)s.own_end) {
            export_dir = k0c < (int)s.own_begin ? 0 : 1;
            exported = true;
            marching = false;
            continue;
        }
        if (f.o000 != cell0 || f.o111 != cell7) {
            cell0 = f.o000;
            cell7 = f.o111;
            c000 = dist_r[(uint64_t)f.o000 * 4]; c100 = dist_r[(uint64_t)f.o100 * 4];
            c010 = dist_r[(uint64_t)f.o010 * 4]; c110 = dist_r[(uint64_t)f.o110 * 4];
            c001 = dist_r[(uint64_t)f.o001 * 4]; c101 = dist_r[(uint64_t)f.o101 * 4];
            c011 = dist_r[(uint64_t)f.o011 * 4]; c111 = dist_r[(uint64_t)f.o111 * 4];
        }
        const float sample_dist = trilerp(c000, c100, c010, c110, c001, c101, c011, c111, f.ax, f.ay, f.az) - 1e-1f;
        ++i;
        if (sample_dist < 1e-5f) {
            status = 1;
            steps = i;
            hit_fp = f;
            marching = false;
        } else {
            dist_from_origin += sample_dist;
            ray_pos = madd(ray_pos, ray_dir, sample_dist);
        }
    }
    if (__ballot(exported) != 0ull) {
        const uint32_t lane = __lane_id();
#pragma unroll
        for (int dir = 0; dir < 2; ++dir) {
            const uint64_t m = __ballot(exported && export_dir == dir);
            if (m == 0ull) continue;
            const uint32_t n = (uint32_t)__popcll(m);
            const int leader = __ffsll((long long)m) - 1;
            uint32_t base = 0;
            if ((int)lane == leader) {
                base = atomicAdd(dir == 0 ? s.count_down : s.count_up, n);
                if (base + n > s.capacity && s.overflow) *s.overflow = 1u;
                if (s.leftover) atomicAdd(s.leftover, n);
            }
            base = __shfl(base, leader);
            const uint32_t at = base + (uint32_t)__popcll(m & ((1ull << lane) - 1ull));
            if (exported && export_dir == dir && at < s.capacity) {
                sdfv_ray_state st;
                st.pixel = pixel;
                st.iteration = (uint32_t)i;
                st.pos[0] = ray_pos.x; st.pos[1] = ray_pos.y; st.pos[2] = ray_pos.z;
                st.t = dist_from_origin;
                (dir == 0 ? s.out_down : s.out_up)[at] = st;
            }
        }
    }
    if (!mine || exported) return;
    if (status == 0) {
        status = -1;
        steps = i;
    }

    float4 rgba = make_float4(0.0f, 0.0f, 0.0f, 0.0f);
    float4 raw0 = rgba, raw1 = rgba;
    if (status == 1) {
        raw0 = gather_rgba(a.tex0, hit_fp);
        raw1 = gather_rgba(a.tex1, hit_fp);
        rgba = shade(a.rp, raw0, raw1);
    }
    a.rgba[pixel] = rgba;
    if (AUX) {
        sdfv_march_aux aux;
        aux_clear(aux);
        aux_set_march(aux, status, steps, ray_pos, dist_from_origin);
        if (status == 1) {
            const float depth = frag_depth_of(cam.bvp, ray_pos.x, ray_pos.y, ray_pos.z);
            aux_set_hit(aux, raw0, raw1, mk(0.0f, 0.0f, 0.0f), depth);
            if (a.fast_normal) {
                const float h = tap_distance((float)tex.w, (float)tex.h, (float)tex.d, a.rp.lod_dist_between_samples);
                const V3 taps[4] = {normal_tap(ray_pos, h, 0), normal_tap(ray_pos, h, 1), normal_tap(ray_pos, h, 2), normal_tap(ray_pos, h, 3)};
                float d[4];
                bool resident = true;
#pragma unroll
                for (int k = 0; k < 4; ++k) {
                    const V3 q = to_p01<XF>(a, taps[k]);
                    const float w = q.z * (float)tex.d - 0.5f;
                    const int k0 = (int)floorf(w);
                    const int lo = max(k0, 0), hi = min(k0 + 1, tex.d - 1);
                    resident = resident && lo >= (int)s.z_lo && hi < (int)(s.z_lo + s.z_count);
                    d[k] = 0.0f;
                    if (resident) {
                        d[k] = gather_r(dist_r, 4, footprint<kClampSlab>(tex, q)) - 1e-1f;
                    }
                }
                if (resident) aux_set_hit(aux, raw0, raw1, normal_of_taps(d[0], d[1], d[2], d[3]), depth);
            }
        }
        a.aux[pixel] = aux;
    }
}

bool asm_addressing_ok(const RaymarchArgs& a) {
    return a.rp.tex_size[0] < (1u << 20) && (uint64_t)a.rp.tex_size[1] * a.rp.tex_size[2] < (1ull << 24);
}

bool hand_written_loop_applies(const RaymarchArgs& a) {
    return a.rp.lod_dist_between_samples == 1.0f && a.fast_index && a.pow2_extent && a.pow2_size && a.symmetric_box && a.asm_loop &&
           a.rp.tex_size[0] >= 2 && asm_addressing_ok(a);
}

bool volume_fits_loop(const RaymarchArgs& a, int mode) {
    const uint64_t texels = (uint64_t)a.rp.tex_size[0] * a.rp.tex_size[1] * a.rp.tex_size[2];
    switch (mode) {
    case kMarchTex0:
    case kMarchPairs: return texels <= (1ull << 28);
    case kMarchDist: return texels <= (1ull << 30);
    case kMarchIlv: return a.rp.tex_size[1] >= 2 && (a.rp.tex_size[1] & 1u) == 0 && texels <= (1ull << 30);
    default: return false;
    }
}

}

bool march_volume_applicable(const RaymarchArgs& a, int kind) {
    return (kind == kMarchPairs || kind == kMarchIlv) && hand_written_loop_applies(a) && volume_fits_loop(a, kind);
}

int march_volume_choice(const RaymarchArgs& a, bool have_dist, bool have_pairs, bool have_ilv) {
    const uint64_t texels = (uint64_t)a.rp.tex_size[0] * a.rp.tex_size[1] * a.rp.tex_size[2];
    const bool cubic = a.rp.tex_size[0] == a.rp.tex_size[1] && a.rp.tex_size[1] == a.rp.tex_size[2];
    if (!cubic && have_dist) return 0;
    const bool pairs_ok = have_pairs && march_volume_applicable(a, kMarchPairs);
    const bool ilv_ok = have_ilv && march_volume_applicable(a, kMarchIlv);
    if (pairs_ok && ilv_ok) return (a.last_level_cache_bytes && texels * 8u > a.last_level_cache_bytes) ? kMarchIlv : kMarchPairs;
    return ilv_ok ? kMarchIlv : (pairs_ok ? kMarchPairs : 0);
}

namespace {
constexpr uint32_t kStoreChunk = 32;
struct CameraChunk {
    sdfv_camera c[kStoreChunk];
};
static_assert(sizeof(sdfv_camera) % 4 == 0, "cameras are copied word by word");
__global__ __launch_bounds__(256) void store_cameras_kernel(CameraChunk chunk, uint32_t words, uint32_t* __restrict__ out) {
    const uint32_t* src = reinterpret_cast<const uint32_t*>(&chunk);
    for (uint32_t w = threadIdx.x; w < words; w += 256) out[w] = src[w];
}
}

hipError_t launch_store_cameras(const sdfv_camera* host, uint32_t n, sdfv_camera* device, hipStream_t stream) {
    for (uint32_t c0 = 0; c0 < n; c0 += kStoreChunk) {
        const uint32_t nc = n - c0 < kStoreChunk ? n - c0 : kStoreChunk;
        CameraChunk chunk;
        memcpy(chunk.c, host + c0, nc * sizeof(sdfv_camera));
        hipLaunchKernelGGL(store_cameras_kernel, dim3(1), dim3(256), 0, stream, chunk, (uint32_t)(nc * sizeof(sdfv_camera) / 4),
                           reinterpret_cast<uint32_t*>(device + c0));
        if (hipError_t e = hipGetLastError()) return e;
    }
    return hipSuccess;
}

hipError_t launch_raymarch_slab(const RaymarchArgs& a, const SlabMarchArgs& s, hipStream_t stream) {
    const bool device_counts = s.in_count[0] || s.in_count[1];
    const uint64_t threads = device_counts ? (uint64_t)s.max_in
                             : s.in ? (uint64_t)s.n_in
                                    : (uint64_t)((a.width + 7) / 8) * ((a.height + 7) / 8) * 64;
    if (threads == 0) return hipSuccess;
    const dim3 grid((uint32_t)((threads + 255) / 256));
    if (a.pow2_extent) {
        if (a.aux) hipLaunchKernelGGL((raymarch_slab_kernel<1, true>), grid, dim3(256), 0, stream, a, s);
        else hipLaunchKernelGGL((raymarch_slab_kernel<1, false>), grid, dim3(256), 0, stream, a, s);
    } else {
        if (a.aux) hipLaunchKernelGGL((raymarch_slab_kernel<0, true>), grid, dim3(256), 0, stream, a, s);
        else hipLaunchKernelGGL((raymarch_slab_kernel<0, false>), grid, dim3(256), 0, stream, a, s);
    }
    return hipGetLastError();
}

namespace {

int march_volume_mode(const RaymarchArgs& a) { return march_volume_choice(a, a.dist != nullptr, a.pairs != nullptr, a.ilv != nullptr); }

struct MarchKernel {
    int mode;
    bool linear;
    int xf;
    bool symm;
    bool hand_written_loop;
};

MarchKernel select_march_kernel(const RaymarchArgs& a, uint32_t lod_filter) {
    MarchKernel k{kMarchGeneral, a.rp.lod_dist_between_samples == 1.0f, a.pow2_extent ? 1 : 0, false, false};
    if (!k.linear && lod_filter == 1) k.mode = kMarchLattice;
    if (!k.linear || !a.fast_index) return k;
    k.mode = march_volume_mode(a);
    if (k.mode == 0) k.mode = a.dist ? kMarchDist : kMarchTex0;
    if (a.pow2_extent && a.pow2_size) k.xf = 2;
    k.symm = k.xf >= 1 && a.symmetric_box;
    k.hand_written_loop = hand_written_loop_applies(a) && volume_fits_loop(a, k.mode);
    return k;
}

template <int MODE, bool LINEAR, int XF, bool SYMM, bool ASM>
void launch_variant(const RaymarchArgs& a, dim3 grid, hipStream_t stream) {
    if (a.aux)
        hipLaunchKernelGGL((raymarch_kernel<MODE, LINEAR, XF, SYMM, true, ASM>), grid, dim3(256), a.lds_cap_bytes, stream, a);
    else if (a.compute_normal)
        hipLaunchKernelGGL((raymarch_kernel<MODE, LINEAR, XF, SYMM, false, ASM, true>), grid, dim3(256), a.lds_cap_bytes, stream, a);
    else
        hipLaunchKernelGGL((raymarch_kernel<MODE, LINEAR, XF, SYMM, false, ASM>), grid, dim3(256), a.lds_cap_bytes, stream, a);
}

constexpr int variant_key(int mode, bool linear, int xf, bool symm, bool hand_written_loop) {
    return mode | (linear ? 8 : 0) | (xf << 4) | (symm ? 64 : 0) | (hand_written_loop ? 128 : 0);
}

hipError_t launch_selected(const MarchKernel& k, const RaymarchArgs& a, dim3 grid, hipStream_t stream) {
#define SDFV_VARIANT(MODE, LINEAR, XF, SYMM, ASM) \
    case variant_key(MODE, LINEAR, XF, SYMM, ASM): launch_variant<MODE, LINEAR, XF, SYMM, ASM>(a, grid, stream); break
    switch (variant_key(k.mode, k.linear, k.xf, k.symm, k.hand_written_loop)) {
        SDFV_VARIANT(kMarchIlv, true, 2, true, true);
        SDFV_VARIANT(kMarchPairs, true, 2, true, true);
        SDFV_VARIANT(kMarchDist, true, 2, true, true);
        SDFV_VARIANT(kMarchDist, true, 2, true, false);
        SDFV_VARIANT(kMarchDist, true, 2, false, false);
        SDFV_VARIANT(kMarchDist, true, 1, true, false);
        SDFV_VARIANT(kMarchDist, true, 1, false, false);
        SDFV_VARIANT(kMarchDist, true, 0, false, false);
        SDFV_VARIANT(kMarchTex0, true, 2, true, true);
        SDFV_VARIANT(kMarchTex0, true, 2, true, false);
        SDFV_VARIANT(kMarchTex0, true, 2, false, false);
        SDFV_VARIANT(kMarchTex0, true, 1, true, false);
        SDFV_VARIANT(kMarchTex0, true, 1, false, false);
        SDFV_VARIANT(kMarchTex0, true, 0, false, false);
        SDFV_VARIANT(kMarchGeneral, true, 1, false, false);
        SDFV_VARIANT(kMarchGeneral, true, 0, false, false);
        SDFV_VARIANT(kMarchGeneral, false, 1, false, false);
        SDFV_VARIANT(kMarchGeneral, false, 0, false, false);
        SDFV_VARIANT(kMarchLattice, false, 1, false, false);
        SDFV_VARIANT(kMarchLattice, false, 0, false, false);
    default: return hipErrorInvalidValue;
    }
#undef SDFV_VARIANT
    return hipGetLastError();
}

}

static void box_first_rectangle(RaymarchArgs& ag, uint32_t groups_y) {
    const sdfv_camera& cam = ag.cameras[0];
    float x_lo = 3.0e38f, x_hi = -3.0e38f, y_lo = 3.0e38f, y_hi = -3.0e38f;
    for (int c = 0; c < 8; ++c) {
        const float p[3] = {(c & 1 ? ag.rp.bounds_max : ag.rp.bounds_min)[0], (c & 2 ? ag.rp.bounds_max : ag.rp.bounds_min)[1],
                            (c & 4 ? ag.rp.bounds_max : ag.rp.bounds_min)[2]};
        const float v[3] = {p[0] - cam.eye[0], p[1] - cam.eye[1], p[2] - cam.eye[2]};
        const float zc = v[0] * cam.forward[0] + v[1] * cam.forward[1] + v[2] * cam.forward[2];
        if (!(zc > 1e-6f)) return;
        const float xc = v[0] * cam.right[0] + v[1] * cam.right[1] + v[2] * cam.right[2];
        const float yc = v[0] * cam.up[0] + v[1] * cam.up[1] + v[2] * cam.up[2];
        const float px = (xc / (zc * cam.aspect * cam.tan_half_fovy) + 1.0f) * 0.5f * (float)ag.width;
        const float py = (1.0f - yc / (zc * cam.tan_half_fovy)) * 0.5f * (float)ag.height - (float)ag.y0;
        if (!(px == px) || !(py == py)) return;
        x_lo = fminf(x_lo, px), x_hi = fmaxf(x_hi, px), y_lo = fminf(y_lo, py), y_hi = fmaxf(y_hi, py);
    }
    const float edge = (float)(16u << ag.group_shift), gxs = (float)ag.groups_x, gys = (float)groups_y;
    const float fx0 = fminf(fmaxf(floorf((x_lo - 1.0f) / edge), 0.0f), gxs), fx1 = fminf(fmaxf(floorf((x_hi + 1.0f) / edge) + 1.0f, 0.0f), gxs);
    const float fy0 = fminf(fmaxf(floorf((y_lo - 1.0f) / edge), 0.0f), gys), fy1 = fminf(fmaxf(floorf((y_hi + 1.0f) / edge) + 1.0f, 0.0f), gys);
    if (!(fx1 > fx0) || !(fy1 > fy0)) return;
    ag.first_gx0 = (uint32_t)fx0, ag.first_gy0 = (uint32_t)fy0;
    ag.first_w = (uint32_t)(fx1 - fx0), ag.first_h = (uint32_t)(fy1 - fy0);
    if (ag.first_w == ag.groups_x && ag.first_h == groups_y) {
        ag.first_w = 0;
        return;
    }
    auto magic = [](uint32_t d) { return d <= 1 ? 0u : (uint32_t)(((1ull << 32) + d - 1) / d); };
    ag.m_groups_x = magic(ag.groups_x), ag.m_first_w = magic(ag.first_w), ag.m_rest_w = magic(ag.groups_x - ag.first_w);
}

static uint32_t occupancy_rule(const RaymarchArgs& ag) {
    if (ag.waves_per_simd >= 2 && ag.waves_per_simd <= 6) return ag.waves_per_simd;
    if (ag.waves_per_simd == 7) return 7;
    if (ag.n_cameras != 1 || ag.first_w == 0 || ag.group_shift == 0 || ag.wave_slots_per_simd_unit == 0) return 7;
    const uint64_t texels = (uint64_t)ag.rp.tex_size[0] * ag.rp.tex_size[1] * ag.rp.tex_size[2];
    const int mode = march_volume_mode(ag);
    const uint64_t volume_bytes = texels * (mode == kMarchPairs ? 8u : ((mode == kMarchIlv || ag.dist) ? 4u : 16u));
    if (ag.last_level_cache_bytes == 0 || volume_bytes <= ag.last_level_cache_bytes) return 7;
    const uint64_t rect_waves = (uint64_t)ag.first_w * ag.first_h * (4ull << (2 * ag.group_shift));
    const uint64_t slots7 = 7ull * ag.wave_slots_per_simd_unit;
    if (rect_waves < slots7 || 2 * rect_waves > 7 * slots7) return 7;
    return 4;
}

static uint32_t lds_cap_for(uint32_t w) {
    uint32_t bytes = (w >= 2 && w <= 6) ? (160u * 1024u) / w - 1024u : 0u;
    if (bytes > 65536u) bytes = 65536u;
    return bytes;
}

hipError_t launch_raymarch(const RaymarchArgs& a, hipStream_t stream, uint32_t lod_filter) {
    const uint32_t rows = a.rows_out;
    if (a.width == 0 || rows == 0 || a.n_cameras == 0) return hipSuccess;
    dim3 grid((a.width + 15) / 16, (rows + 15) / 16, a.n_cameras);
    RaymarchArgs ag = a;
    const dim3 tiles = grid;
#ifdef SDFV_TUNING
    if (a.tile_order) {
        ag.group_shift = 0;
        ag.lds_cap_bytes = lds_cap_for(occupancy_rule(ag));
        return launch_selected(select_march_kernel(ag, lod_filter), ag, dim3(tiles.x * tiles.y, 1, 1), stream);
    }
#endif
    auto grouped = [&](uint32_t shift) {
        ag.group_shift = shift;
        ag.tiles_x = tiles.x;
        ag.tiles_y = tiles.y;
        ag.groups_x = (tiles.x + (1u << shift) - 1) >> shift;
        const uint32_t groups_y = (tiles.y + (1u << shift) - 1) >> shift;
        const uint32_t groups = ((ag.groups_x * groups_y + 7u) / 8u) * 8u;
        ag.first_w = 0;
        if (a.box_first && a.n_cameras == 1 && groups < 65536u) box_first_rectangle(ag, groups_y);
        grid = dim3(groups << (2 * shift), 1, a.n_cameras);
    };
    if (a.band_skip) {
        ag.group_shift = 0;
    } else if (a.group_shift == kGroupAuto) {
        grouped(1);
        if (ag.first_w == 0) grouped(2);
    } else if (a.group_shift) {
        grouped(a.group_shift);
    }
    ag.lds_cap_bytes = lds_cap_for(occupancy_rule(ag));
    return launch_selected(select_march_kernel(ag, lod_filter), ag, grid, stream);
}

}
```

Baseline: 204,000.

## Trim hand-written march loop: packed weights, single-compare cube OOB, restructured fetch

Reworks the inline-asm sphere-trace loop. The cube out-of-bounds test now uses one max3 on absolute coordinates against a precomputed float limit instead of subtract-then-compare. The trilinear weight computation switches to packed ops with a constant 1.0 pair held in scalar registers, and the fetch paths share a common exit sequence. The goal is fewer VALU instructions per march step, at the cost of a new host-side threshold helper that must exactly reproduce the old epsilon comparison and extra scalar register clobbers.

```diff
diff --git a/profiles/march_loop_trim/raymarch_loop_hand_box.s b/profiles/march_loop_trim/raymarch_loop_hand_box.s
--- /dev/null
+++ b/profiles/march_loop_trim/raymarch_loop_hand_box.s
@@ -0,0 +1,148 @@
+s_mov_b64 s[76:77], exec
+s_and_b64 exec, exec, s[14:15]
+s_cbranch_execz .Ldone_17
+s_mov_b32 s66, s5
+s_mov_b32 s67, s6
+s_mov_b32 s70, s37
+s_mov_b32 s71, s41
+s_mov_b32 s72, 0xbf000000
+s_mov_b32 s73, 0xbf000000
+s_mov_b32 s88, 1.0
+s_mov_b32 s89, 1.0
+s_add_i32 s75, s40, -1
+s_lshl_b32 s82, s10, 2
+s_lshl_b32 s83, s10, 4
+s_lshl_b32 s85, s10, 3
+s_movk_i32 s74, 254
+s_mov_b32 s64, s82
+s_mul_i32 s86, s38, s82
+s_add_u32 s68, s2, s86
+s_addc_u32 s69, s3, 0
+s_add_u32 s64, s2, s64
+s_addc_u32 s65, s3, 0
+s_add_u32 s86, s64, s86
+s_addc_u32 s87, s65, 0
+v_mov_b32 v68, 0x7f800000
+v_mov_b32 v70, 0x7f800000
+v_mov_b32 v71, 0x7f800000
+.Lloop_17:
+v_sub_f32_e64 v32, |v40|, s7
+v_subrev_f32_e32 v48, s4, v40
+v_sub_f32_e64 v33, |v42|, s8
+v_pk_add_f32 v[50:51], v[42:43], s[66:67] neg_lo:[0,1] neg_hi:[0,1]
+v_sub_f32_e64 v34, |v43|, s9
+v_mul_f32_e32 v48, s36, v48
+v_pk_mul_f32 v[50:51], v[50:51], s[70:71]
+v_max3_f32 v32, v32, v33, v34
+v_add_f32_e32 v48, -0.5, v48
+v_pk_add_f32 v[50:51], v[50:51], s[72:73]
+v_cmpx_nlt_f32_e32 vcc, s13, v32
+v_sub_f32_e32 v52, v48, v68
+v_pk_add_f32 v[54:55], v[50:51], v[70:71] neg_lo:[0,1] neg_hi:[0,1]
+v_max3_u32 v32, v52, v54, v55
+v_cmp_gt_u32_e32 vcc, 0x3f800000, v32
+s_cbranch_execz .Ldone_17
+s_andn2_b64 vcc, exec, vcc
+s_cbranch_scc1 .Lfetch_17
+.Lcached_17:
+v_sub_f32_e32 v53, 1.0, v52
+v_pk_add_f32 v[56:57], s[88:89], v[54:55] neg_lo:[0,1] neg_hi:[0,1]
+v_pk_mul_f32 v[34:35], v[62:63], v[52:53] op_sel_hi:[1,0]
+v_pk_mul_f32 v[38:39], v[66:67], v[52:53] op_sel_hi:[1,0]
+v_pk_mul_f32 v[32:33], v[60:61], v[52:53] op_sel:[0,1] op_sel_hi:[1,1]
+v_pk_mul_f32 v[36:37], v[64:65], v[52:53] op_sel:[0,1] op_sel_hi:[1,1]
+v_pk_add_f32 v[32:33], v[32:33], v[34:35]
+v_pk_add_f32 v[36:37], v[36:37], v[38:39]
+v_pk_mul_f32 v[32:33], v[32:33], v[56:57] op_sel_hi:[1,0]
+v_pk_mul_f32 v[36:37], v[36:37], v[54:55] op_sel_hi:[1,0]
+v_pk_add_f32 v[32:33], v[32:33], v[36:37]
+v_mul_f32_e32 v32, v32, v57
+v_mul_f32_e32 v33, v33, v55
+v_add_f32_e32 v36, v32, v33
+v_add_f32_e32 v36, 0xbdcccccd, v36
+v_cmpx_ngt_f32_e32 vcc, 0x3727c5ac, v36
+v_mul_f32_e32 v32, v44, v36
+v_pk_mul_f32 v[34:35], v[46:47], v[36:37] op_sel_hi:[1,0]
+v_add_f32_e32 v40, v40, v32
+v_pk_add_f32 v[42:43], v[42:43], v[34:35]
+s_add_u32 s74, s74, -1
+s_cbranch_scc1 .Lloop_17
+s_branch .Ldone_17
+.Lfetch_17:
+s_and_saveexec_b64 s[78:79], vcc
+v_floor_f32_e32 v68, v48
+v_floor_f32_e32 v70, v50
+v_floor_f32_e32 v71, v51
+v_cvt_i32_f32_e32 v32, v68
+v_cvt_i32_f32_e32 v33, v70
+v_cvt_i32_f32_e32 v34, v71
+v_max3_u32 v35, v32, v33, v34
+v_cmp_gt_u32_e32 vcc, s39, v35
+s_xor_b64 vcc, vcc, exec
+s_cbranch_scc1 .Lborder_17
+v_mad_u32_u24 v39, v34, s38, v33
+v_mad_u32_u24 v39, v39, s10, v32
+v_lshlrev_b32_e32 v39, 2, v39
+global_load_dwordx2 v[24:25], v39, s[2:3]
+global_load_dwordx2 v[26:27], v39, s[64:65]
+global_load_dwordx2 v[28:29], v39, s[68:69]
+global_load_dwordx2 v[30:31], v39, s[86:87]
+v_sub_f32_e32 v52, v48, v68
+v_pk_add_f32 v[54:55], v[50:51], v[70:71] neg_lo:[0,1] neg_hi:[0,1]
+s_waitcnt vmcnt(1)
+v_pk_mov_b32 v[60:61], v[24:25], v[28:29] op_sel:[0,0]
+v_pk_mov_b32 v[62:63], v[24:25], v[28:29] op_sel:[1,1]
+s_waitcnt vmcnt(0)
+v_pk_mov_b32 v[64:65], v[26:27], v[30:31] op_sel:[0,0]
+v_pk_mov_b32 v[66:67], v[26:27], v[30:31] op_sel:[1,1]
+s_mov_b64 exec, s[78:79]
+s_branch .Lcached_17
+.Lborder_17:
+v_sub_f32_e32 v52, v48, v68
+v_pk_add_f32 v[54:55], v[50:51], v[70:71] neg_lo:[0,1] neg_hi:[0,1]
+v_max_i32_e32 v35, 0, v32
+v_max_i32_e32 v37, 0, v33
+v_max_i32_e32 v38, 0, v34
+v_add_u32_e32 v32, 1, v32
+v_add_u32_e32 v33, 1, v33
+v_add_u32_e32 v34, 1, v34
+v_min_i32_e32 v32, s40, v32
+v_min_i32_e32 v33, s33, v33
+v_min_i32_e32 v34, s19, v34
+v_mad_u32_u24 v28, v38, s38, v37
+v_mad_u32_u24 v29, v38, s38, v33
+v_mad_u32_u24 v30, v34, s38, v37
+v_mad_u32_u24 v31, v34, s38, v33
+v_min_i32_e32 v36, s75, v35
+v_lshlrev_b32_e32 v39, 2, v36
+v_mad_u32_u24 v28, v28, s82, v39
+v_mad_u32_u24 v29, v29, s82, v39
+v_mad_u32_u24 v30, v30, s82, v39
+v_mad_u32_u24 v31, v31, s82, v39
+global_load_dwordx2 v[24:25], v28, s[2:3]
+global_load_dwordx2 v[26:27], v29, s[2:3]
+global_load_dwordx2 v[28:29], v30, s[2:3]
+global_load_dwordx2 v[30:31], v31, s[2:3]
+v_cmp_eq_u32_e64 s[80:81], v35, v36
+v_add_u32_e32 v36, 1, v36
+v_cmp_eq_u32_e32 vcc, v32, v36
+s_waitcnt vmcnt(3)
+v_cndmask_b32_e64 v60, v25, v24, s[80:81]
+v_cndmask_b32_e32 v62, v24, v25, vcc
+s_waitcnt vmcnt(2)
+v_cndmask_b32_e64 v64, v27, v26, s[80:81]
+v_cndmask_b32_e32 v66, v26, v27, vcc
+s_waitcnt vmcnt(1)
+v_cndmask_b32_e64 v61, v29, v28, s[80:81]
+v_cndmask_b32_e32 v63, v28, v29, vcc
+s_waitcnt vmcnt(0)
+v_cndmask_b32_e64 v65, v31, v30, s[80:81]
+v_cndmask_b32_e32 v67, v30, v31, vcc
+s_mov_b64 exec, s[78:79]
+s_branch .Lcached_17
+.Ldone_17:
+s_mov_b64 s[22:23], exec
+s_mov_b32 s12, s74
+s_and_b64 exec, s[76:77], s[14:15]
+s_nop 0
+s_mov_b64 exec, s[76:77]
diff --git a/profiles/march_loop_trim/raymarch_loop_hand_cube.s b/profiles/march_loop_trim/raymarch_loop_hand_cube.s
--- /dev/null
+++ b/profiles/march_loop_trim/raymarch_loop_hand_cube.s
@@ -0,0 +1,145 @@
+s_mov_b64 s[76:77], exec
+s_and_b64 exec, exec, s[14:15]
+s_cbranch_execz .Ldone_16
+s_mov_b32 s66, s5
+s_mov_b32 s67, s6
+s_mov_b32 s70, s37
+s_mov_b32 s71, s41
+s_mov_b32 s72, 0xbf000000
+s_mov_b32 s73, 0xbf000000
+s_mov_b32 s88, 1.0
+s_mov_b32 s89, 1.0
+s_add_i32 s75, s40, -1
+s_lshl_b32 s82, s10, 2
+s_lshl_b32 s83, s10, 4
+s_lshl_b32 s85, s10, 3
+s_movk_i32 s74, 254
+s_mov_b32 s64, s82
+s_mul_i32 s86, s38, s82
+s_add_u32 s68, s2, s86
+s_addc_u32 s69, s3, 0
+s_add_u32 s64, s2, s64
+s_addc_u32 s65, s3, 0
+s_add_u32 s86, s64, s86
+s_addc_u32 s87, s65, 0
+v_mov_b32 v68, 0x7f800000
+v_mov_b32 v70, 0x7f800000
+v_mov_b32 v71, 0x7f800000
+.Lloop_16:
+v_max3_f32 v32, |v40|, |v42|, |v43|
+v_subrev_f32_e32 v48, s4, v40
+v_pk_add_f32 v[50:51], v[42:43], s[66:67] neg_lo:[0,1] neg_hi:[0,1]
+v_mul_f32_e32 v48, s36, v48
+v_pk_mul_f32 v[50:51], v[50:51], s[70:71]
+v_add_f32_e32 v48, -0.5, v48
+v_pk_add_f32 v[50:51], v[50:51], s[72:73]
+v_cmpx_nlt_f32_e32 vcc, s13, v32
+v_sub_f32_e32 v52, v48, v68
+v_pk_add_f32 v[54:55], v[50:51], v[70:71] neg_lo:[0,1] neg_hi:[0,1]
+v_max3_u32 v32, v52, v54, v55
+v_cmp_gt_u32_e32 vcc, 0x3f800000, v32
+s_cbranch_execz .Ldone_16
+s_andn2_b64 vcc, exec, vcc
+s_cbranch_scc1 .Lfetch_16
+.Lcached_16:
+v_sub_f32_e32 v53, 1.0, v52
+v_pk_add_f32 v[56:57], s[88:89], v[54:55] neg_lo:[0,1] neg_hi:[0,1]
+v_pk_mul_f32 v[34:35], v[62:63], v[52:53] op_sel_hi:[1,0]
+v_pk_mul_f32 v[38:39], v[66:67], v[52:53] op_sel_hi:[1,0]
+v_pk_mul_f32 v[32:33], v[60:61], v[52:53] op_sel:[0,1] op_sel_hi:[1,1]
+v_pk_mul_f32 v[36:37], v[64:65], v[52:53] op_sel:[0,1] op_sel_hi:[1,1]
+v_pk_add_f32 v[32:33], v[32:33], v[34:35]
+v_pk_add_f32 v[36:37], v[36:37], v[38:39]
+v_pk_mul_f32 v[32:33], v[32:33], v[56:57] op_sel_hi:[1,0]
+v_pk_mul_f32 v[36:37], v[36:37], v[54:55] op_sel_hi:[1,0]
+v_pk_add_f32 v[32:33], v[32:33], v[36:37]
+v_mul_f32_e32 v32, v32, v57
+v_mul_f32_e32 v33, v33, v55
+v_add_f32_e32 v36, v32, v33
+v_add_f32_e32 v36, 0xbdcccccd, v36
+v_cmpx_ngt_f32_e32 vcc, 0x3727c5ac, v36
+v_mul_f32_e32 v32, v44, v36
+v_pk_mul_f32 v[34:35], v[46:47], v[36:37] op_sel_hi:[1,0]
+v_add_f32_e32 v40, v40, v32
+v_pk_add_f32 v[42:43], v[42:43], v[34:35]
+s_add_u32 s74, s74, -1
+s_cbranch_scc1 .Lloop_16
+s_branch .Ldone_16
+.Lfetch_16:
+s_and_saveexec_b64 s[78:79], vcc
+v_floor_f32_e32 v68, v48
+v_floor_f32_e32 v70, v50
+v_floor_f32_e32 v71, v51
+v_cvt_i32_f32_e32 v32, v68
+v_cvt_i32_f32_e32 v33, v70
+v_cvt_i32_f32_e32 v34, v71
+v_max3_u32 v35, v32, v33, v34
+v_cmp_gt_u32_e32 vcc, s39, v35
+s_xor_b64 vcc, vcc, exec
+s_cbranch_scc1 .Lborder_16
+v_mad_u32_u24 v39, v34, s38, v33
+v_mad_u32_u24 v39, v39, s10, v32
+v_lshlrev_b32_e32 v39, 2, v39
+global_load_dwordx2 v[24:25], v39, s[2:3]
+global_load_dwordx2 v[26:27], v39, s[64:65]
+global_load_dwordx2 v[28:29], v39, s[68:69]
+global_load_dwordx2 v[30:31], v39, s[86:87]
+v_sub_f32_e32 v52, v48, v68
+v_pk_add_f32 v[54:55], v[50:51], v[70:71] neg_lo:[0,1] neg_hi:[0,1]
+s_waitcnt vmcnt(1)
+v_pk_mov_b32 v[60:61], v[24:25], v[28:29] op_sel:[0,0]
+v_pk_mov_b32 v[62:63], v[24:25], v[28:29] op_sel:[1,1]
+s_waitcnt vmcnt(0)
+v_pk_mov_b32 v[64:65], v[26:27], v[30:31] op_sel:[0,0]
+v_pk_mov_b32 v[66:67], v[26:27], v[30:31] op_sel:[1,1]
+s_mov_b64 exec, s[78:79]
+s_branch .Lcached_16
+.Lborder_16:
+v_sub_f32_e32 v52, v48, v68
+v_pk_add_f32 v[54:55], v[50:51], v[70:71] neg_lo:[0,1] neg_hi:[0,1]
+v_max_i32_e32 v35, 0, v32
+v_max_i32_e32 v37, 0, v33
+v_max_i32_e32 v38, 0, v34
+v_add_u32_e32 v32, 1, v32
+v_add_u32_e32 v33, 1, v33
+v_add_u32_e32 v34, 1, v34
+v_min_i32_e32 v32, s40, v32
+v_min_i32_e32 v33, s33, v33
+v_min_i32_e32 v34, s19, v34
+v_mad_u32_u24 v28, v38, s38, v37
+v_mad_u32_u24 v29, v38, s38, v33
+v_mad_u32_u24 v30, v34, s38, v37
+v_mad_u32_u24 v31, v34, s38, v33
+v_min_i32_e32 v36, s75, v35
+v_lshlrev_b32_e32 v39, 2, v36
+v_mad_u32_u24 v28, v28, s82, v39
+v_mad_u32_u24 v29, v29, s82, v39
+v_mad_u32_u24 v30, v30, s82, v39
+v_mad_u32_u24 v31, v31, s82, v39
+global_load_dwordx2 v[24:25], v28, s[2:3]
+global_load_dwordx2 v[26:27], v29, s[2:3]
+global_load_dwordx2 v[28:29], v30, s[2:3]
+global_load_dwordx2 v[30:31], v31, s[2:3]
+v_cmp_eq_u32_e64 s[80:81], v35, v36
+v_add_u32_e32 v36, 1, v36
+v_cmp_eq_u32_e32 vcc, v32, v36
+s_waitcnt vmcnt(3)
+v_cndmask_b32_e64 v60, v25, v24, s[80:81]
+v_cndmask_b32_e32 v62, v24, v25, vcc
+s_waitcnt vmcnt(2)
+v_cndmask_b32_e64 v64, v27, v26, s[80:81]
+v_cndmask_b32_e32 v66, v26, v27, vcc
+s_waitcnt vmcnt(1)
+v_cndmask_b32_e64 v61, v29, v28, s[80:81]
+v_cndmask_b32_e32 v63, v28, v29, vcc
+s_waitcnt vmcnt(0)
+v_cndmask_b32_e64 v65, v31, v30, s[80:81]
+v_cndmask_b32_e32 v67, v30, v31, vcc
+s_mov_b64 exec, s[78:79]
+s_branch .Lcached_16
+.Ldone_16:
+s_mov_b64 s[42:43], exec
+s_mov_b32 s12, s74
+s_and_b64 exec, s[76:77], s[14:15]
+s_nop 0
+s_mov_b64 exec, s[76:77]
diff --git a/profiles/march_loop_trim/raymarch_loop_hipcc.s b/profiles/march_loop_trim/raymarch_loop_hipcc.s
--- /dev/null
+++ b/profiles/march_loop_trim/raymarch_loop_hipcc.s
@@ -0,0 +1,167 @@
+.LBB16_42:
+	v_mov_b32_e32 v0, v28
+	v_mov_b32_e32 v31, v29
+	v_mov_b32_e32 v32, v30
+.LBB16_43:
+	s_or_b64 exec, exec, s[44:45]
+.LBB16_44:
+	s_or_b64 exec, exec, s[42:43]
+	v_sub_f32_e32 v28, v25, v28
+	v_sub_f32_e32 v34, v27, v30
+	v_sub_f32_e32 v30, 1.0, v28
+	s_waitcnt vmcnt(2)
+	v_pk_mul_f32 v[36:37], v[28:29], v[16:17] op_sel_hi:[0,1]
+	v_pk_mul_f32 v[40:41], v[30:31], v[14:15] op_sel_hi:[0,1]
+	v_sub_f32_e32 v26, v26, v29
+	s_waitcnt vmcnt(0)
+	v_pk_mul_f32 v[28:29], v[28:29], v[20:21] op_sel_hi:[0,1]
+	v_pk_add_f32 v[36:37], v[36:37], v[40:41]
+	v_pk_mul_f32 v[40:41], v[30:31], v[18:19] op_sel_hi:[0,1]
+	v_sub_f32_e32 v38, 1.0, v26
+	v_pk_add_f32 v[28:29], v[28:29], v[40:41]
+	v_pk_mul_f32 v[36:37], v[38:39], v[36:37] op_sel_hi:[0,1]
+	v_pk_mul_f32 v[26:27], v[26:27], v[28:29] op_sel_hi:[0,1]
+	v_sub_f32_e32 v35, 1.0, v34
+	v_pk_add_f32 v[26:27], v[26:27], v[36:37]
+	s_add_i32 s50, s50, -1
+	v_pk_mul_f32 v[26:27], v[34:35], v[26:27]
+	s_nop 0
+	v_add_f32_e32 v25, v26, v27
+	v_add_f32_e32 v26, 0xbdcccccd, v25
+	v_cmp_ngt_f32_e32 vcc, s49, v26
+	s_and_b64 s[2:3], s[40:41], vcc
+	v_pk_mul_f32 v[28:29], v[2:3], v[26:27] op_sel_hi:[1,0]
+	v_mul_f32_e32 v25, v7, v26
+	s_cmp_eq_u32 s50, 0
+	v_pk_add_f32 v[28:29], v[8:9], v[28:29]
+	v_add_f32_e32 v25, v6, v25
+	s_cselect_b64 s[40:41], -1, 0
+	s_andn2_b64 s[38:39], s[38:39], exec
+	s_and_b64 s[42:43], s[2:3], exec
+	v_cndmask_b32_e64 v9, v9, v29, s[2:3]
+	v_cndmask_b32_e64 v8, v8, v28, s[2:3]
+	v_cndmask_b32_e64 v6, v6, v25, s[2:3]
+	s_or_b64 s[38:39], s[38:39], s[42:43]
+	s_and_b64 vcc, exec, s[40:41]
+	s_cbranch_vccnz .LBB16_55
+.LBB16_45:
+	s_mov_b64 s[40:41], 0
+	s_and_saveexec_b64 s[42:43], s[2:3]
+	v_sub_f32_e64 v25, |v8|, s7
+	v_sub_f32_e64 v26, |v9|, s8
+	v_sub_f32_e64 v27, |v6|, s9
+	v_max3_f32 v25, v25, v26, v27
+	v_cmp_nlt_f32_e32 vcc, s48, v25
+	s_and_b64 s[40:41], vcc, exec
+	s_or_b64 exec, exec, s[42:43]
+	v_cndmask_b32_e64 v25, 0, 1, s[40:41]
+	s_andn2_b64 s[2:3], s[38:39], exec
+	s_and_b64 s[38:39], s[40:41], exec
+	v_cmp_ne_u32_e32 vcc, 0, v25
+	s_or_b64 s[38:39], s[2:3], s[38:39]
+	s_cbranch_vccz .LBB16_54
+	v_subrev_f32_e32 v25, s4, v8
+	v_subrev_f32_e32 v26, s5, v9
+	v_subrev_f32_e32 v27, s6, v6
+	v_mul_f32_e32 v25, v22, v25
+	v_mul_f32_e32 v26, v23, v26
+	v_mul_f32_e32 v27, v24, v27
+	v_add_f32_e32 v25, -0.5, v25
+	v_add_f32_e32 v26, -0.5, v26
+	v_add_f32_e32 v27, -0.5, v27
+	v_floor_f32_e32 v28, v25
+	v_floor_f32_e32 v29, v26
+	v_floor_f32_e32 v30, v27
+	s_and_saveexec_b64 s[42:43], s[40:41]
+	s_cbranch_execz .LBB16_44
+	v_cmp_neq_f32_e32 vcc, v28, v0
+	v_cmp_neq_f32_e64 s[2:3], v29, v31
+	s_or_b64 s[2:3], vcc, s[2:3]
+	v_cmp_neq_f32_e32 vcc, v30, v32
+	s_or_b64 s[2:3], s[2:3], vcc
+	s_and_saveexec_b64 s[44:45], s[2:3]
+	s_cbranch_execz .LBB16_43
+	v_cvt_i32_f32_e32 v0, v28
+	v_cvt_i32_f32_e32 v14, v29
+	v_cvt_i32_f32_e32 v15, v30
+	s_mov_b64 s[2:3], -1
+	v_max_i32_e32 v31, 0, v0
+	v_add_u32_e32 v0, 1, v0
+	v_min_i32_e32 v32, s46, v0
+	v_max_i32_e32 v0, 0, v14
+	v_add_u32_e32 v14, 1, v14
+	v_max_i32_e32 v16, 0, v15
+	v_add_u32_e32 v15, 1, v15
+	v_min_i32_e32 v14, s33, v14
+	v_min_i32_e32 v15, s11, v15
+	v_mul_lo_u32 v0, v0, s10
+	v_mul_lo_u32 v14, v14, s10
+	v_mul_lo_u32 v16, v16, s19
+	v_mul_lo_u32 v15, v15, s19
+	v_add_u32_e32 v36, v0, v16
+	v_add_u32_e32 v35, v14, v16
+	v_add_u32_e32 v34, v15, v0
+	v_add_u32_e32 v33, v14, v15
+	s_and_b64 vcc, exec, s[36:37]
+	s_cbranch_vccz .LBB16_52
+	v_add_u32_e32 v0, v36, v31
+	v_lshl_add_u64 v[38:39], v[0:1], 2, s[34:35]
+	v_add_u32_e32 v0, v36, v32
+	v_lshl_add_u64 v[40:41], v[0:1], 2, s[34:35]
+	v_add_u32_e32 v0, v35, v31
+	v_lshl_add_u64 v[42:43], v[0:1], 2, s[34:35]
+	v_add_u32_e32 v0, v35, v32
+	v_lshl_add_u64 v[44:45], v[0:1], 2, s[34:35]
+	v_add_u32_e32 v0, v34, v31
+	v_lshl_add_u64 v[46:47], v[0:1], 2, s[34:35]
+	v_add_u32_e32 v0, v34, v32
+	v_lshl_add_u64 v[48:49], v[0:1], 2, s[34:35]
+	v_add_u32_e32 v0, v33, v31
+	v_lshl_add_u64 v[50:51], v[0:1], 2, s[34:35]
+	v_add_u32_e32 v0, v33, v32
+	v_lshl_add_u64 v[52:53], v[0:1], 2, s[34:35]
+	global_load_dword v15, v[38:39], off
+	global_load_dword v17, v[40:41], off
+	global_load_dword v19, v[42:43], off
+	global_load_dword v21, v[44:45], off
+	global_load_dword v14, v[46:47], off
+	global_load_dword v16, v[48:49], off
+	global_load_dword v18, v[50:51], off
+	global_load_dword v20, v[52:53], off
+	s_mov_b64 s[2:3], 0
+.LBB16_52:
+	s_andn2_b64 vcc, exec, s[2:3]
+	s_cbranch_vccnz .LBB16_42
+	v_min_u32_e32 v38, s47, v31
+	v_add_u32_e32 v0, v36, v38
+	s_waitcnt vmcnt(3)
+	v_lshl_add_u64 v[14:15], v[0:1], 2, s[34:35]
+	v_add_u32_e32 v0, v35, v38
+	global_load_dwordx2 v[16:17], v[14:15], off
+	v_lshl_add_u64 v[14:15], v[0:1], 2, s[34:35]
+	v_add_u32_e32 v0, v34, v38
+	s_waitcnt vmcnt(2)
+	v_lshl_add_u64 v[18:19], v[0:1], 2, s[34:35]
+	v_add_u32_e32 v0, v33, v38
+	global_load_dwordx2 v[20:21], v[14:15], off
+	global_load_dwordx2 v[34:35], v[18:19], off
+	v_lshl_add_u64 v[14:15], v[0:1], 2, s[34:35]
+	global_load_dwordx2 v[36:37], v[14:15], off
+	v_add_u32_e32 v0, 1, v38
+	v_cmp_lt_u32_e32 vcc, s47, v31
+	v_cmp_eq_u32_e64 s[2:3], v32, v0
+	s_waitcnt vmcnt(3)
+	v_cndmask_b32_e32 v15, v16, v17, vcc
+	v_cndmask_b32_e64 v17, v16, v17, s[2:3]
+	s_waitcnt vmcnt(2)
+	v_cndmask_b32_e32 v19, v20, v21, vcc
+	v_cndmask_b32_e64 v21, v20, v21, s[2:3]
+	s_waitcnt vmcnt(1)
+	v_cndmask_b32_e32 v14, v34, v35, vcc
+	v_cndmask_b32_e64 v16, v34, v35, s[2:3]
+	s_waitcnt vmcnt(0)
+	v_cndmask_b32_e32 v18, v36, v37, vcc
+	v_cndmask_b32_e64 v20, v36, v37, s[2:3]
+	s_branch .LBB16_42
+.LBB16_54:
+	s_cbranch_execz .LBB16_45
diff --git a/sdf-viewer_amd/csrc/api_march.hip b/sdf-viewer_amd/csrc/api_march.hip
--- a/sdf-viewer_amd/csrc/api_march.hip
+++ b/sdf-viewer_amd/csrc/api_march.hip
@@ -4,6 +4,7 @@
 
 #include "api_internal.h"
 #include "march_common.h"
+#include "march_threshold.h"
 #include "raymarch_kernels.h"
 
 using namespace sdfv;
@@ -122,6 +123,7 @@
     a.asm_loop = (off & SDFV_RM_NO_ASM_LOOP) ? 0u : 1u;
     a.no_interior_fetch = (off & SDFV_RM_NO_INTERIOR_FETCH) ? 1u : 0u;
     a.cube_box = (a.symmetric_box && rp->bounds_max[0] == rp->bounds_max[1] && rp->bounds_max[1] == rp->bounds_max[2]) ? 1u : 0u;
+    a.oob_limit = a.cube_box ? sdfv::march::oob_threshold(rp->bounds_max[0], 1e-4f) : 1e-4f;
     if (off & SDFV_RM_NO_SYMMETRIC) a.symmetric_box = 0;
     if (off & SDFV_RM_NO_POW2_SIZE) a.pow2_size = 0;
 }
diff --git a/sdf-viewer_amd/csrc/march_threshold.h b/sdf-viewer_amd/csrc/march_threshold.h
--- /dev/null
+++ b/sdf-viewer_amd/csrc/march_threshold.h
@@ -0,0 +1,16 @@
+#pragma once
+
+#include <math.h>
+
+namespace sdfv {
+namespace march {
+
+inline float oob_threshold(float m, float eps) {
+    float x = m + eps;
+    while (x - m > eps) x = nextafterf(x, -INFINITY);
+    for (float up = nextafterf(x, INFINITY); up - m <= eps; up = nextafterf(x, INFINITY)) x = up;
+    return x;
+}
+
+}
+}
diff --git a/sdf-viewer_amd/csrc/raymarch_kernels.h b/sdf-viewer_amd/csrc/raymarch_kernels.h
--- a/sdf-viewer_amd/csrc/raymarch_kernels.h
+++ b/sdf-viewer_amd/csrc/raymarch_kernels.h
@@ -39,6 +39,7 @@
     uint32_t wave_slots_per_simd_unit;
     uint64_t last_level_cache_bytes;
     uint32_t cube_box;
+    float oob_limit;
     uint32_t rows_out;
     uint32_t band_skip;
     uint32_t band_shift;
diff --git a/sdf-viewer_amd/csrc/raymarch_kernels.hip b/sdf-viewer_amd/csrc/raymarch_kernels.hip
--- a/sdf-viewer_amd/csrc/raymarch_kernels.hip
+++ b/sdf-viewer_amd/csrc/raymarch_kernels.hip
@@ -300,6 +300,7 @@
     "s_mov_b32 s66, %[miny]\n s_mov_b32 s67, %[minz]\n"                                            \
     "s_mov_b32 s70, %[ky]\n s_mov_b32 s71, %[kz]\n"                                                    \
     "s_mov_b32 s72, 0xbf000000\n s_mov_b32 s73, 0xbf000000\n"                                      \
+    "s_mov_b32 s88, 1.0\n s_mov_b32 s89, 1.0\n"                                                         \
     "s_add_i32 s75, %[wm1], -1\n"                                                                         \
     "s_lshl_b32 s82, %[w], 2\n s_lshl_b32 s83, %[w], 4\n"         \
     "s_lshl_b32 s85, %[w], 3\n"                                      \
@@ -317,8 +318,7 @@
 #define SDFV_MARCH_ASM_OOB4_B "v_sub_f32_e64 v33, |v42|, %[my]\n"
 #define SDFV_MARCH_ASM_OOB4_C "v_sub_f32_e64 v34, |v43|, %[mz]\n"
 #define SDFV_MARCH_ASM_OOB4_D "v_max3_f32 v32, v32, v33, v34\n"
-#define SDFV_MARCH_ASM_OOB2_A "v_max3_f32 v32, |v40|, |v42|, |v43|\n"
-#define SDFV_MARCH_ASM_OOB2_D "v_subrev_f32_e32 v32, %[mx], v32\n"
+#define SDFV_MARCH_ASM_OOB1_A "v_max3_f32 v32, |v40|, |v42|, |v43|\n"
 #define SDFV_MARCH_ASM_TOP(T_STEP, OOB_A, OOB_B, OOB_C, OOB_D)                                                      \
     OOB_A                                                                                                           \
     "v_subrev_f32_e32 v48, %[minx], v40\n"                                                                          \
@@ -330,32 +330,34 @@
     OOB_D                                                                                                           \
     "v_add_f32_e32 v48, -0.5, v48\n"                                                                                \
     "v_pk_add_f32 v[50:51], v[50:51], s[72:73]\n"                                                                   \
-    "v_cmpx_nlt_f32_e32 vcc, 0x38d1b717, v32\n"                                           \
-    "s_cbranch_execz .Ldone_%=\n"                                                                                   \
-    "v_sub_f32_e32 v52, v48, v68\n"                                                                              \
-    "v_sub_f32_e32 v54, v50, v70\n"                                                                              \
-    "v_sub_f32_e32 v56, v51, v71\n" T_STEP                                                                       \
-    "v_max3_u32 v32, v52, v54, v56\n"                                                                            \
-    "v_cmp_gt_u32_e32 vcc, 0x3f800000, v32\n"                                                                       \
-    "s_andn1_saveexec_b64 s[78:79], vcc\n"                                      \
-    "s_cbranch_execnz .Lfetch_%=\n"                                  \
+    "v_cmpx_nlt_f32_e32 vcc, %[lim], v32\n"                   \
+          \
+    "v_sub_f32_e32 v52, v48, v68\n"                                                                                 \
+    "v_pk_add_f32 v[54:55], v[50:51], v[70:71] neg_lo:[0,1] neg_hi:[0,1]\n" T_STEP                                 \
+    "v_max3_u32 v32, v52, v54, v55\n"                                                                               \
+    "v_cmp_gt_u32_e32 vcc, 0x3f800000, v32\n"                   \
+    "s_cbranch_execz .Ldone_%=\n"                             \
+    "s_andn2_b64 vcc, exec, vcc\n"                                  \
+    "s_cbranch_scc1 .Lfetch_%=\n"                                    \
     ".Lcached_%=:\n"
+#define SDFV_MARCH_ASM_WEIGHTS                                \
+    "v_sub_f32_e32 v52, v48, v68\n v_pk_add_f32 v[54:55], v[50:51], v[70:71] neg_lo:[0,1] neg_hi:[0,1]\n"
+#define SDFV_MARCH_ASM_FETCH_END "s_mov_b64 exec, s[78:79]\n s_branch .Lcached_%=\n"
 #define SDFV_MARCH_ASM_FETCH_PREP(INTERIOR)                                                                         \
     ".Lfetch_%=:\n"                                                                                                 \
+    "s_and_saveexec_b64 s[78:79], vcc\n"                      \
     SDFV_MARCH_ASM_TUNE("s_add_u32 s84, s84, 1\n")                                                                  \
-        \
+                                       \
     "v_floor_f32_e32 v68, v48\n v_floor_f32_e32 v70, v50\n v_floor_f32_e32 v71, v51\n"                         \
     "v_cvt_i32_f32_e32 v32, v68\n v_cvt_i32_f32_e32 v33, v70\n v_cvt_i32_f32_e32 v34, v71\n"                      \
-    "v_sub_f32_e32 v52, v48, v68\n v_sub_f32_e32 v54, v50, v70\n v_sub_f32_e32 v56, v51, v71\n"             \
      \
     "v_max3_u32 v35, v32, v33, v34\n"                                                                               \
     "v_cmp_gt_u32_e32 vcc, %[thresh], v35\n"                                                                        \
     "s_xor_b64 vcc, vcc, exec\n"                                                                                    \
     "s_cbranch_scc1 .Lborder_%=\n"                                                                                  \
     "v_mad_u32_u24 v39, v34, %[h], v33\n"                     \
-    "v_mad_u32_u24 v39, v39, %[w], v32\n" INTERIOR                                                               \
-    "s_branch .Lcached_%=\n"                                                                                        \
-    ".Lborder_%=:\n"                                                                                                \
+    "v_mad_u32_u24 v39, v39, %[w], v32\n" INTERIOR SDFV_MARCH_ASM_FETCH_END                                       \
+    ".Lborder_%=:\n" SDFV_MARCH_ASM_WEIGHTS                                                                        \
     "v_max_i32_e32 v35, 0, v32\n v_max_i32_e32 v37, 0, v33\n v_max_i32_e32 v38, 0, v34\n"         \
     "v_add_u32_e32 v32, 1, v32\n v_add_u32_e32 v33, 1, v33\n v_add_u32_e32 v34, 1, v34\n"                            \
     "v_min_i32_e32 v32, %[wm1], v32\n v_min_i32_e32 v33, %[hm1], v33\n v_min_i32_e32 v34, %[dm1], v34\n"   \
@@ -369,6 +371,7 @@
     "global_load_dwordx2 v[26:27], v39, s[64:65]\n"                                       \
     "global_load_dwordx2 v[28:29], v39, s[68:69]\n"                                       \
     "global_load_dwordx2 v[30:31], v39, s[86:87]\n"                                       \
+    SDFV_MARCH_ASM_WEIGHTS                                                                                          \
     "s_waitcnt vmcnt(1)\n"                                                                                          \
     "v_pk_mov_b32 v[60:61], v[24:25], v[28:29] op_sel:[0,0]\n"                                    \
     "v_pk_mov_b32 v[62:63], v[24:25], v[28:29] op_sel:[1,1]\n"                                    \
@@ -381,11 +384,13 @@
     "global_load_dword v64, v39, s[64:65]\n global_load_dword v66, v39, s[64:65] offset:16\n"                     \
     "global_load_dword v61, v39, s[68:69]\n global_load_dword v63, v39, s[68:69] offset:16\n"                     \
     "global_load_dword v65, v39, s[86:87]\n global_load_dword v67, v39, s[86:87] offset:16\n"                     \
+    SDFV_MARCH_ASM_WEIGHTS                                                                                          \
     "s_waitcnt vmcnt(0)\n"
 #define SDFV_MARCH_ASM_INTERIOR_PAIRS                                                                               \
     "v_lshlrev_b32_e32 v39, 3, v39\n"                                                                               \
     "global_load_dwordx4 v[24:27], v39, %[base]\n"                                  \
     "global_load_dwordx4 v[28:31], v39, s[68:69]\n"                                 \
+    SDFV_MARCH_ASM_WEIGHTS                                                                                          \
     "s_waitcnt vmcnt(0)\n"                                                                                          \
     "v_pk_mov_b32 v[60:61], v[24:25], v[28:29] op_sel:[0,0]\n"                                    \
     "v_pk_mov_b32 v[64:65], v[24:25], v[28:29] op_sel:[1,1]\n"                                    \
@@ -401,24 +406,24 @@
     "global_load_dword v61, v24, %[base]\n global_load_dword v63, v25, %[base]\n"                                  \
     "v_mad_u32_u24 v26, v31, s85, v35\n v_mad_u32_u24 v27, v31, s85, v32\n"                                          \
     "global_load_dword v65, v26, %[base]\n global_load_dword v67, v27, %[base]\n"                                  \
-    "s_waitcnt vmcnt(0)\n"                                                                                          \
-    "s_branch .Lcached_%=\n"
+    "s_waitcnt vmcnt(0)\n" SDFV_MARCH_ASM_FETCH_END
 #define SDFV_MARCH_ASM_INTERIOR_ILV                                                                                 \
     "s_lshr_b32 s80, %[h], 1\n"                                                                                     \
-    "v_and_b32_e32 v48, 1, v33\n"                                                                  \
+    "v_and_b32_e32 v31, 1, v33\n"                                                                  \
     "v_lshrrev_b32_e32 v35, 1, v33\n"                                                              \
     "v_add_u32_e32 v36, 1, v33\n"                                                                                   \
     "v_lshrrev_b32_e32 v36, 1, v36\n"                                                        \
     "v_mad_u32_u24 v35, v34, s80, v35\n v_mad_u32_u24 v36, v34, s80, v36\n"              \
     "v_mad_u32_u24 v35, v35, %[w], v32\n v_mad_u32_u24 v37, v36, %[w], v32\n"                                        \
     "v_lshlrev_b32_e32 v36, 3, v35\n v_lshlrev_b32_e32 v37, 3, v37\n"                                               \
-    "v_cmp_eq_u32_e32 vcc, 1, v48\n"                                                                                \
+    "v_cmp_eq_u32_e32 vcc, 1, v31\n"                                                                                \
     "global_load_dwordx4 v[24:27], v36, %[base]\n"                      \
     "global_load_dwordx4 v[32:35], v36, s[68:69]\n"                                                      \
     "s_and_saveexec_b64 s[80:81], vcc\n"                      \
     "global_load_dwordx3 v[28:30], v37, %[base]\n"                                   \
     "global_load_dwordx3 v[36:38], v37, s[68:69]\n"                                                      \
     "s_mov_b64 exec, s[80:81]\n"                                                                                    \
+    SDFV_MARCH_ASM_WEIGHTS                                                                                          \
     "s_waitcnt vmcnt(2)\n"                                                                                          \
     "v_cndmask_b32_e32 v60, v24, v25, vcc\n v_cndmask_b32_e32 v62, v26, v27, vcc\n"          \
     "v_cndmask_b32_e32 v61, v32, v33, vcc\n v_cndmask_b32_e32 v63, v34, v35, vcc\n"                  \
@@ -441,8 +446,7 @@
     "global_load_dword v61, v24, %[base]\n global_load_dword v63, v25, %[base]\n"                                  \
     "v_add_u32_e32 v26, v31, v35\n v_add_u32_e32 v27, v31, v32\n"                                                    \
     "global_load_dword v65, v26, %[base]\n global_load_dword v67, v27, %[base]\n"                                  \
-    "s_waitcnt vmcnt(0)\n"                                                                                          \
-    "s_branch .Lcached_%=\n"
+    "s_waitcnt vmcnt(0)\n" SDFV_MARCH_ASM_FETCH_END
 #define SDFV_MARCH_ASM_FETCH_DIST                                                                                   \
     "v_min_i32_e32 v36, s75, v35\n"                                                         \
     "v_lshlrev_b32_e32 v39, 2, v36\n"                                                                               \
@@ -463,7 +467,7 @@
     "v_cndmask_b32_e64 v61, v29, v28, s[80:81]\n v_cndmask_b32_e32 v63, v28, v29, vcc\n"           \
     "s_waitcnt vmcnt(0)\n"                                                                                          \
     "v_cndmask_b32_e64 v65, v31, v30, s[80:81]\n v_cndmask_b32_e32 v67, v30, v31, vcc\n"           \
-    "s_branch .Lcached_%=\n"
+    SDFV_MARCH_ASM_FETCH_END
 #define SDFV_MARCH_ASM_FETCH_TEX0                                                                                   \
     "v_lshlrev_b32_e32 v35, 4, v35\n v_lshlrev_b32_e32 v32, 4, v32\n"                  \
     "v_mad_u32_u24 v24, v28, s83, v35\n v_mad_u32_u24 v25, v28, s83, v32\n"                                          \
@@ -474,11 +478,10 @@
     "global_load_dword v61, v24, %[base]\n global_load_dword v63, v25, %[base]\n"                                  \
     "v_mad_u32_u24 v26, v31, s83, v35\n v_mad_u32_u24 v27, v31, s83, v32\n"                                          \
     "global_load_dword v65, v26, %[base]\n global_load_dword v67, v27, %[base]\n"                                  \
-    "s_waitcnt vmcnt(0)\n"                                                                                          \
-    "s_branch .Lcached_%=\n"
+    "s_waitcnt vmcnt(0)\n" SDFV_MARCH_ASM_FETCH_END
 #define SDFV_MARCH_ASM_FILTER                                                                                       \
-    "s_mov_b64 exec, s[78:79]\n"                                                                                    \
-    "v_sub_f32_e32 v53, 1.0, v52\n v_sub_f32_e32 v55, 1.0, v54\n v_sub_f32_e32 v57, 1.0, v56\n"                \
+    "v_sub_f32_e32 v53, 1.0, v52\n"                                                                                 \
+    "v_pk_add_f32 v[56:57], s[88:89], v[54:55] neg_lo:[0,1] neg_hi:[0,1]\n"                                         \
                                                                 \
     "v_pk_mul_f32 v[34:35], v[62:63], v[52:53] op_sel_hi:[1,0]\n"                                                \
     "v_pk_mul_f32 v[38:39], v[66:67], v[52:53] op_sel_hi:[1,0]\n"                                                \
@@ -487,11 +490,12 @@
     "v_pk_add_f32 v[32:33], v[32:33], v[34:35]\n"                                                    \
     "v_pk_add_f32 v[36:37], v[36:37], v[38:39]\n"                                                    \
                                                                                                    \
-    "v_pk_mul_f32 v[32:33], v[32:33], v[54:55] op_sel:[0,1] op_sel_hi:[1,1]\n"                                     \
-    "v_pk_mul_f32 v[36:37], v[36:37], v[54:55] op_sel_hi:[1,0]\n"                                                  \
+    "v_pk_mul_f32 v[32:33], v[32:33], v[56:57] op_sel_hi:[1,0]\n"                                   \
+    "v_pk_mul_f32 v[36:37], v[36:37], v[54:55] op_sel_hi:[1,0]\n"                                         \
     "v_pk_add_f32 v[32:33], v[32:33], v[36:37]\n"                                                      \
                                                                        \
-    "v_pk_mul_f32 v[32:33], v[32:33], v[56:57] op_sel:[0,1] op_sel_hi:[1,0]\n"       \
+    "v_mul_f32_e32 v32, v32, v57\n"                                                              \
+    "v_mul_f32_e32 v33, v33, v55\n"                                \
     "v_add_f32_e32 v36, v32, v33\n"                                                                                 \
     "v_add_f32_e32 v36, 0xbdcccccd, v36\n"                                                                          \
                                                                                  \
@@ -516,11 +520,11 @@
 #define SDFV_MARCH_ASM_OPERANDS                                                                                     \
     [dx] "v"(dirx), [dy] "v"(diry), [dz] "v"(dirz), [cov] "s"(cov), [mx] "s"(a.rp.bounds_max[0]),    \
         [my] "s"(a.rp.bounds_max[1]), [mz] "s"(a.rp.bounds_max[2]), [minx] "s"(a.rp.bounds_min[0]),                 \
-        [miny] "s"(a.rp.bounds_min[1]), [minz] "s"(a.rp.bounds_min[2]), [kx] "s"(kx), [ky] "s"(ky), [kz] "s"(kz),   \
+        [miny] "s"(a.rp.bounds_min[1]), [minz] "s"(a.rp.bounds_min[2]), [lim] "s"(a.oob_limit), [kx] "s"(kx), [ky] "s"(ky), [kz] "s"(kz), \
         [wm1] "s"(wm1), [hm1] "s"(hm1), [dm1] "s"(dm1), [w] "s"(t.w), [h] "s"(t.h), [base] "s"(vol), [base_lo] "s"(base_lo), [base_hi] "s"(base_hi), [thresh] "s"(thresh)
 #define SDFV_MARCH_ASM_CLOBBERS                                                                                     \
     "vcc", "scc", "memory", "s64", "s65", "s66", "s67", "s68", "s69", "s70", "s71", "s72", "s73", "s74", "s75",    \
-        "s76", "s77", "s78", "s79", "s80", "s81", "s82", "s83", "s84", "s85", "s86", "s87", "v24", "v25", "v26", "v27", "v28",  \
+        "s76", "s77", "s78", "s79", "s80", "s81", "s82", "s83", "s84", "s85", "s86", "s87", "s88", "s89", "v24", "v25", "v26", "v27", "v28",  \
         "v29", "v30", "v31", "v32", "v33", "v34", "v35", "v36", "v37", "v38", "v39", "v48", "v50", "v51", "v52",    \
         "v53", "v54", "v55", "v56", "v57", "v58", "v59", "v60", "v61", "v62", "v63", "v64", "v65", "v66", "v67", "v68",   \
         "v70", "v71"
@@ -545,7 +549,7 @@
     register float diry asm("v46") = ray_dir.y;
     register float dirz asm("v47") = ray_dir.z;
 #define SDFV_MARCH_ASM_OOB_BOX SDFV_MARCH_ASM_OOB4_A, SDFV_MARCH_ASM_OOB4_B, SDFV_MARCH_ASM_OOB4_C, SDFV_MARCH_ASM_OOB4_D
-#define SDFV_MARCH_ASM_OOB_CUBE SDFV_MARCH_ASM_OOB2_A, "", "", SDFV_MARCH_ASM_OOB2_D
+#define SDFV_MARCH_ASM_OOB_CUBE SDFV_MARCH_ASM_OOB1_A, "", "", ""
 #define SDFV_MARCH_ASM_TOP_(T_STEP, ...) SDFV_MARCH_ASM_TOP(T_STEP, __VA_ARGS__)
 #define SDFV_MARCH_ASM_RUN_AUX(SHIFT, INTERIOR, FETCH, OOB)                                                         \
     asm volatile("v_mov_b32 v58, %[tt]\n v_mov_b32 v59, 0\n" SDFV_MARCH_ASM_HEAD(SHIFT)                             \
```

After: 204,100, median of 3. About the same (+0.0%).
